# deepika090/HL-HGAT

Hardware: AMD Instinct MI355X
Metric: graphs/sec HL-HGAT fwd+bwd, ZINC-12k simplex graphs, 1/2/4/8 MI355X (higher is better)
Workload: dtype fp32; 1 GPU; BASELINE configs[1]: ZINC-12k-scale, HL_HGCNN_zinc_dense_int3_pyr channels=[2,2,2] filters=[64,64,64] K=3 mlp=[256,256] keig=15; step = copy of the device-resident batch into the step's static buffers + fwd + L1 + bwd (+ grad all-reduce) + Adam; the batch tables (Laplacian / incidence CSRs, degrees, segment offsets) are built by the data loader at collate time, outside the step (see loader); graphs_per_gpu=1000, global_batch=1000, parallelism=dp1

## Files before the change

hl-hgat_amd/csrc/collate.hip:

```cpp
#include <cstdint>
#include <cstring>
#include <vector>

#include "common.h"

namespace {

struct Sizes {
  int64_t n_t = 0, n_s = 0, z_t = 0, z_s = 0;
};

int batch_sizes(const hlhgat_packed_graphs_t* d, const int64_t* idx, int64_t B, Sizes& s) {
  for (int64_t b = 0; b < B; ++b) {
    const int64_t g = idx[b];
    HLH_CHECK_ARG(g >= 0 && g < d->n_graphs, "collate: graph id %lld out of range [0, %lld)",
                  (long long)g, (long long)d->n_graphs);
    s.n_t += d->node_ptr[g + 1] - d->node_ptr[g];
    s.n_s += d->edge_ptr[g + 1] - d->edge_ptr[g];
    s.z_t += d->lt_ptr[g + 1] - d->lt_ptr[g];
    s.z_s += d->ls_ptr[g + 1] - d->ls_ptr[g];
  }
  return HLHGAT_OK;
}

void pad_loops(int64_t n, int64_t R, int64_t z, int64_t Z, int64_t* row, int64_t* col,
               float* w) {
  const int64_t extra = Z - z, bins = R - n;
  if (extra <= 0 || bins <= 0) return;
  const int64_t base = extra / bins, more = extra % bins;
  int64_t p = z;
  for (int64_t r = n; r < R; ++r) {
    const int64_t k = base + (r - n < more ? 1 : 0);
    for (int64_t i = 0; i < k; ++i, ++p) {
      row[p] = r;
      col[p] = r;
      w[p] = 0.f;
    }
  }
}

void coo_csr(const int64_t* row, const int64_t* col, int64_t nnz, int64_t n, int32_t* rowptr,
             int32_t* ccol) {
  std::memset(rowptr, 0, sizeof(int32_t) * (size_t)(n + 1));
  for (int64_t e = 0; e < nnz; ++e) rowptr[row[e] + 1]++;
  for (int64_t r = 0; r < n; ++r) rowptr[r + 1] += rowptr[r];
  for (int64_t e = 0; e < nnz; ++e) ccol[e] = (int32_t)col[e];
}

}

extern "C" int hlhgat_collate_sizes(const hlhgat_packed_graphs_t* d, const int64_t* idx,
                                    int64_t n_idx, int64_t* sizes) {
  HLH_CHECK_ARG(d && sizes && n_idx >= 0 && (n_idx == 0 || idx), "collate_sizes: bad arguments");
  Sizes s;
  const int rc = batch_sizes(d, idx, n_idx, s);
  if (rc) return rc;
  sizes[0] = s.n_t;
  sizes[1] = s.n_s;
  sizes[2] = s.z_t;
  sizes[3] = s.z_s;
  return HLHGAT_OK;
}

extern "C" int hlhgat_collate(const hlhgat_packed_graphs_t* d, const int64_t* idx, int64_t B,
                              hlhgat_collated_t* o) {
  HLH_CHECK_ARG(d && o && B > 0 && idx, "collate: bad arguments");
  HLH_CHECK_ARG(d->node_ptr && d->edge_ptr && d->lt_ptr && d->ls_ptr && d->x_t && d->x_s &&
                    d->lt_row && d->lt_col && d->lt_w && d->ls_row && d->ls_col && d->ls_w &&
                    d->b1_src && d->b1_dst && d->f_t > 0 && d->f_s > 0 &&
                    (d->y_dim == 0 || d->y),
                "collate: incomplete packed dataset");
  Sizes s;
  int rc = batch_sizes(d, idx, B, s);
  if (rc) return rc;
  const int64_t Rt = o->rows_t, Rs = o->rows_s, Zt = o->nnz_t, Zs = o->nnz_s;
  const bool padded = !(Rt == s.n_t && Rs == s.n_s && Zt == s.z_t && Zs == s.z_s);
  if (padded)
    HLH_CHECK_ARG(Rt > s.n_t && Rs > s.n_s && Zt >= s.z_t && Zs >= s.z_s,
                  "collate: capacities (%lld, %lld, %lld, %lld) do not hold the batch "
                  "(%lld, %lld, %lld, %lld)",
                  (long long)Rt, (long long)Rs, (long long)Zt, (long long)Zs,
                  (long long)s.n_t, (long long)s.n_s, (long long)s.z_t, (long long)s.z_s);
  HLH_CHECK_ARG(Rt < INT32_MAX && 2 * Rs < INT32_MAX && Zt < INT32_MAX && Zs < INT32_MAX,
                "collate: batch too large for int32 tables");
  HLH_CHECK_ARG(o->x_t && o->x_s && o->edge_index_t && o->edge_weight_t && o->edge_index_s &&
                    o->edge_weight_s && o->edge_index && o->num_node1 && o->num_edge1 &&
                    (d->y_dim == 0 || o->y),
                "collate: NULL output");
  const int64_t Ft = d->f_t, Fs = d->f_s;
  int64_t* eit_r = o->edge_index_t;
  int64_t* eit_c = o->edge_index_t + Zt;
  int64_t* eis_r = o->edge_index_s;
  int64_t* eis_c = o->edge_index_s + Zs;
  int64_t* b1_r = o->edge_index;
  int64_t* b1_c = o->edge_index + Rs;
  int64_t nt = 0, ns = 0, zt = 0, zs = 0;
  for (int64_t b = 0; b < B; ++b) {
    const int64_t g = idx[b];
    const int64_t n0 = d->node_ptr[g], n1 = d->node_ptr[g + 1];
    const int64_t e0 = d->edge_ptr[g], e1 = d->edge_ptr[g + 1];
    const int64_t t0 = d->lt_ptr[g], t1 = d->lt_ptr[g + 1];
// ... 33 lines not shown
    }
    if (d->y_dim)
      std::memcpy(o->y + b * d->y_dim, d->y + g * d->y_dim, sizeof(float) * (size_t)d->y_dim);
    o->num_node1[b] = n1 - n0;
    o->num_edge1[b] = e1 - e0;
    nt += n1 - n0;
    ns += e1 - e0;
    zt += t1 - t0;
    zs += s1 - s0;
  }
  std::memset(o->x_t + nt * Ft, 0, sizeof(float) * (size_t)((Rt - nt) * Ft));
  std::memset(o->x_s + ns * Fs, 0, sizeof(float) * (size_t)((Rs - ns) * Fs));
  pad_loops(nt, Rt, zt, Zt, eit_r, eit_c, o->edge_weight_t);
  pad_loops(ns, Rs, zs, Zs, eis_r, eis_c, o->edge_weight_s);
  for (int64_t i = 0; i < Rs - ns; ++i) {
    b1_r[ns + i] = nt + i % (Rt - nt);
    b1_c[ns + i] = nt + i % (Rt - nt);
  }
  if (o->csr_rowptr_t && o->csr_col_t) coo_csr(eit_r, eit_c, Zt, Rt, o->csr_rowptr_t, o->csr_col_t);
  if (o->csr_rowptr_s && o->csr_col_s) coo_csr(eis_r, eis_c, Zs, Rs, o->csr_rowptr_s, o->csr_col_s);
  if (o->inc_rowptr && o->inc_eids) {
    int32_t* rp = o->inc_rowptr;
    std::memset(rp, 0, sizeof(int32_t) * (size_t)(Rt + 1));
    for (int64_t e = 0; e < Rs; ++e) {
      HLH_CHECK_ARG(b1_r[e] >= 0 && b1_r[e] < Rt && b1_c[e] >= 0 && b1_c[e] < Rt,
                    "collate: B1 edge %lld out of range", (long long)e);
      rp[b1_r[e] + 1]++;
      rp[b1_c[e] + 1]++;
    }
    for (int64_t r = 0; r < Rt; ++r) rp[r + 1] += rp[r];
    std::vector<int32_t> fill(rp, rp + Rt);
    for (int64_t e = 0; e < Rs; ++e) {
      o->inc_eids[fill[b1_r[e]]++] = (int32_t)e;
      o->inc_eids[fill[b1_c[e]]++] = (int32_t)e;
    }
    if (o->deg_t && o->inv_deg_t) {
      for (int64_t r = 0; r < Rt; ++r) {
        const float dv = (padded && r >= nt) ? 1.f : (float)(rp[r + 1] - rp[r]);
        o->deg_t[r] = dv;
        o->inv_deg_t[r] = 1.f / dv;
      }
    }
  }
  if (o->seg_ptr_t && o->seg_ptr_s) {
    o->seg_ptr_t[0] = 0;
    o->seg_ptr_s[0] = 0;
    for (int64_t b = 0; b < B; ++b) {
      o->seg_ptr_t[b + 1] = o->seg_ptr_t[b] + (int32_t)o->num_node1[b];
      o->seg_ptr_s[b + 1] = o->seg_ptr_s[b] + (int32_t)o->num_edge1[b];
    }
  }
  if (o->valid_mask_t)
    for (int64_t r = 0; r < Rt; ++r) o->valid_mask_t[r] = r < nt ? 1 : 0;
  o->n_t = nt;
  o->n_s = ns;
  return HLHGAT_OK;
}
```

hl-hgat_amd/csrc/poly.hip:

```cpp
#include "common.h"

#include <cstdlib>

using namespace hlhgat;

namespace {

struct PolyArgs {
  const int32_t* order;
  const int32_t* rowptr;
  const int32_t* col;
  const float* val;
  const float* rs;
  const float* X;
  const float* B;
  const float* Z;
  const float* P;
  const float* Q;
  float* Y;
  int64_t ldx, ldb, ldz, ldp, ldq, ldy;
  int64_t n_rows;
  int d;
  float alpha, beta, gamma, div, p, q;
  const int32_t* hdr;
// ... 117 lines not shown
            c[u] = __shfl(cm, j + u, LPR);
            w[u] = __shfl(wm, j + u, LPR);
          }
          if (fok) {
            vt x[8];
#pragma unroll
            for (int u = 0; u < 8; ++u) x[u] = vload<V>(X + (int64_t)c[u] * a.ldx + f);
#pragma unroll
            for (int i = 0; i < V; ++i) {
              float s = vget(acc, i);
#pragma unroll
              for (int u = 0; u < 8; ++u) s = s + w[u] * vget(x[u], i);
              vget(acc, i) = s;
            }
          }
        }
      }
      for (; j + 3 < cnt; j += 4) {
        const int c0 = __shfl(cm, j, LPR), c1 = __shfl(cm, j + 1, LPR),
                  c2 = __shfl(cm, j + 2, LPR), c3 = __shfl(cm, j + 3, LPR);
        const float w0 = __shfl(wm, j, LPR), w1 = __shfl(wm, j + 1, LPR),
                    w2 = __shfl(wm, j + 2, LPR), w3 = __shfl(wm, j + 3, LPR);
        if (fok) {
          vt x0 = vload<V>(X + (int64_t)c0 * a.ldx + f);
          vt x1 = vload<V>(X + (int64_t)c1 * a.ldx + f);
          vt x2 = vload<V>(X + (int64_t)c2 * a.ldx + f);
          vt x3 = vload<V>(X + (int64_t)c3 * a.ldx + f);
#pragma unroll
          for (int i = 0; i < V; ++i) {
            float s = vget(acc, i);
            s = s + w0 * vget(x0, i);
            s = s + w1 * vget(x1, i);
            s = s + w2 * vget(x2, i);
            s = s + w3 * vget(x3, i);
            vget(acc, i) = s;
          }
        }
      }
      if (j < cnt) gather_batch<V, 3, LPR>(X, a.ldx, f, fok, cm, wm, j, cnt - j, acc);
    }
    if (!fok) continue;
    poly_epilogue<V>(a, row, f, acc, rsv);
  }
}

template <int V, int LPR>
__global__ __launch_bounds__(256) void k_poly_step(PolyArgs a) {
  poly_step_body<V, LPR, 4>(a, blk_hw());
}

template <int V, int LPR>
__global__ __launch_bounds__(256) void k_poly_step_deep(PolyArgs a) {
  poly_step_body<V, LPR, 8>(a, blk_hw());
}

template <int V, int LPR>
__global__ __launch_bounds__(256) void k_hodge_edge_step(PolyArgs a) {
  using vt = typename VecT<V>::type;
  constexpr int kEpg = 4;
  const int64_t grp = ((int64_t)xcd_slot(blockIdx.x, gridDim.x) * 256 + threadIdx.x) / LPR;
  const int sub = threadIdx.x % LPR;
  const int64_t s0 = grp * kEpg;
  if (s0 >= a.n_rows) return;
  int64_t e[kEpg];
  int2 ij[kEpg];
  float al[kEpg];
#pragma unroll
  for (int u = 0; u < kEpg; ++u) {
    const int64_t sl = s0 + u < a.n_rows ? s0 + u : s0;
    e[u] = a.order ? (int64_t)a.order[sl] : sl;
  }
#pragma unroll
  for (int u = 0; u < kEpg; ++u) {
    ij[u] = a.ends[e[u]];
    al[u] = a.ealpha[e[u]];
  }
  const float* __restrict__ Z = a.X;
  for (int f = sub * V; f < a.d; f += LPR * V) {
    vt zi[kEpg], zj[kEpg];
#pragma unroll
    for (int u = 0; u < kEpg; ++u) {
      zi[u] = vload<V>(Z + (int64_t)ij[u].x * a.ldx + f);
      zj[u] = vload<V>(Z + (int64_t)ij[u].y * a.ldx + f);
    }
#pragma unroll
    for (int u = 0; u < kEpg; ++u) {
      if (s0 + u >= a.n_rows) break;
      vt acc;
#pragma unroll
      for (int c = 0; c < V; ++c) {
        float s = 0.f;
        s = s + (-al[u]) * vget(zi[u], c);
        s = s + al[u] * vget(zj[u], c);
        vget(acc, c) = s;
      }
      poly_epilogue<V>(a, e[u], f, acc, 1.f);
    }
  }
}

constexpr int kHaloIds = 8;

template <int V, int LPR, int NT>
__global__ __launch_bounds__(NT) void k_poly_halo(PolyArgs a) {
  using vt = typename VecT<V>::type;
  constexpr int FS = V * LPR;
// ... 454 lines not shown
}

int launch_factored(PolyArgs a, const hlhgat_hodge_factor_t& f, float* work, hipStream_t s) {
  HLH_CHECK_ARG(f.node_rowptr && f.ends && f.alpha && work && a.n_rows == f.n_edges &&
                    (f.n_edges == 0 || (f.node_edge && f.node_sign)),
                "hodge factor: incomplete descriptor or row count %lld != n_edges %lld",
                (long long)a.n_rows, (long long)f.n_edges);
  HLH_CHECK_ARG(!a.rs, "hodge factor: row scale not supported");
  if (a.n_rows == 0) return HLHGAT_OK;
  if (a.beta != 0.f && !a.B) {
    a.B = a.X;
    a.ldb = a.ldx;
  }
  {
    PolyArgs b = make_args(f.node_rowptr, f.node_edge, f.node_sign, f.n_nodes, a.X, a.ldx, a.d,
                           work, a.d, f.node_order);
    const double b1 = 16.0 * (double)f.n_edges + 4.0 * (double)(f.n_nodes + 1) +
                      4.0 * (double)(f.n_edges + f.n_nodes) * a.d;
    int rc = launch_poly(b, 2 * f.n_edges, s, HLHGAT_PROF_HODGE_NODE, b1);
    if (rc) return rc;
  }
  a.X = work;
  a.ldx = a.d;
  a.order = f.edge_order;
  a.ends = reinterpret_cast<const int2*>(f.ends);
  a.ealpha = f.alpha;
  a.lcol = nullptr;
  a.n_tiles = 0;
  const int v = pick_vec(a.d, {a.ldx, a.ldy, a.Z ? a.ldz : 4, a.P ? a.ldp : 4, a.Q ? a.ldq : 4,
                               a.B ? a.ldb : 4},
                         {a.X, a.Y, a.Z, a.P, a.Q, a.B});
  const int l = pick_lpr(a.d, v);
  a.nt_store = (double)a.n_rows * a.d * 4.0 >= kNtStoreBytes;
  int dense = 1 + (a.beta != 0.f) + (a.Z != nullptr) + (a.P != nullptr) + (a.Q != nullptr);
  ProfScope prof(HLHGAT_PROF_HODGE_EDGE, s,
                 12.0 * (double)a.n_rows + 4.0 * (double)(f.n_nodes + dense * a.n_rows) * a.d,
                 4.0 * (double)a.n_rows * a.d);
  HLH_DISPATCH_VL(v, l, k_hodge_edge_step, ceil_div(a.n_rows, (int64_t)4), s, a, &prof);
  HLH_CHECK_LAUNCH();
  return HLHGAT_OK;
}

struct StepRunner {
  int64_t nnz;
  const hlhgat_hodge_factor_t* fac;
  float* work;
  hipStream_t s;
  int prof_class = HLHGAT_PROF_POLY;
  int operator()(PolyArgs& a) const {
    return fac ? launch_factored(a, *fac, work, s) : launch_poly(a, nnz, s, prof_class);
  }
};

}

using namespace hlhgat;

extern "C" int hlhgat_spmm(const int32_t* rowptr, const int32_t* col,
                           const float* val, int64_t n_rows, int64_t nnz,
                           const int32_t* row_order, const hlhgat_halo_t* halo,
                           const float* X, int64_t ldx,
                           int64_t d, float* Y, int64_t ldy, void* stream) {
  PolyArgs a = make_args(rowptr, col, val, n_rows, X, ldx, d, Y, ldy, row_order, halo);
  return launch_poly(a, nnz, as_stream(stream));
}

extern "C" int hlhgat_poly_step(const int32_t* rowptr, const int32_t* col,
                                const float* val, const float* rs,
                                int64_t n_rows, int64_t nnz,
                                const int32_t* row_order, const hlhgat_halo_t* halo,
                                const float* X,
                                int64_t ldx, int64_t d, const float* Z,
                                int64_t ldz, const float* P, int64_t ldp,
                                const float* Q, int64_t ldq, float alpha,
                                float beta, float gamma, float div, float p,
                                float q, float* Y, int64_t ldy, void* stream) {
  PolyArgs a = make_args(rowptr, col, val, n_rows, X, ldx, d, Y, ldy, row_order, halo);
  a.rs = rs;
  a.Z = Z;
  a.ldz = ldz;
  a.P = P;
  a.ldp = ldp;
  a.Q = Q;
  a.ldq = ldq;
  a.alpha = alpha;
  a.beta = beta;
  a.gamma = gamma;
  a.div = div;
  a.p = p;
  a.q = q;
  return launch_poly(a, nnz, as_stream(stream));
}

extern "C" int hlhgat_incidence_step(const int32_t* rowptr, const int32_t* col,
                                     const float* val, const float* rs, int64_t n_rows,
                                     int64_t nnz, int64_t n_src, const float* X, int64_t ldx,
                                     int64_t d, const float* Z, int64_t ldz, float alpha,
                                     float gamma, float* Y, int64_t ldy, void* stream) {
  HLH_CHECK_ARG(n_src >= 0, "incidence_step: n_src < 0");
  PolyArgs a = make_args(rowptr, col, val, n_rows, X, ldx, d, Y, ldy);
  a.rs = rs;
  a.Z = Z;
  a.ldz = ldz;
  a.alpha = alpha;
  a.gamma = gamma;
  a.div = 1.f;
  const double bytes = (double)nnz * (val ? 8.0 : 4.0) + 4.0 * (double)(n_rows + 1) +
                       4.0 * (double)n_src * d + 4.0 * (double)n_rows * d * (Z ? 2.0 : 1.0) +
                       (rs ? 4.0 * (double)n_rows : 0.0);
  return launch_poly(a, nnz, as_stream(stream), HLHGAT_PROF_INCIDENCE, bytes);
}

namespace {
int basis_fwd_core(int kind, const int32_t* rowptr, const int32_t* col, const float* val,
                   int64_t n, int64_t nnz, const int32_t* row_order, const hlhgat_halo_t* halo,
                   const float* X, int64_t ldx, int64_t F, int K, float* T,
                   const hlhgat_hodge_factor_t* fac, float* work, void* stream) {
  HLH_CHECK_ARG(kind == HLHGAT_POLY_LAGUERRE || kind == HLHGAT_POLY_CHEB ||
                    kind == HLHGAT_POLY_LAGUERRE_DEMO,
                "poly_basis_fwd: bad kind %d", kind);
  HLH_CHECK_ARG(K >= 1, "poly_basis_fwd: K must be > 0 (assert K > 0)");
  if (K == 1 || n == 0) return HLHGAT_OK;
  HLH_CHECK_ARG(T, "poly_basis_fwd: T is NULL");
  hipStream_t s = as_stream(stream);
  const StepRunner run{nnz, fac, work, s};
  const int64_t blk = n * F;
  auto Tk = [&](int k) -> float* { return T + (int64_t)(k - 1) * blk; };
  {
    PolyArgs a = make_args(rowptr, col, val, n, X, ldx, F, Tk(1), F, row_order, halo);
    if (kind != HLHGAT_POLY_CHEB) {
      a.alpha = -1.f;
      a.beta = 1.f;
    }
    int rc = run(a);
    if (rc) return rc;
  }
  for (int k = 1; k + 1 < K; ++k) {
    const float* prev = (k == 1) ? X : Tk(k - 1);
    const int64_t ldprev = (k == 1) ? ldx : F;
    PolyArgs a = make_args(rowptr, col, val, n, Tk(k), F, F, Tk(k + 1), F, row_order, halo);
    a.Z = prev;
    a.ldz = ldprev;
    if (kind == HLHGAT_POLY_LAGUERRE_DEMO) {
      a.X = X;
      a.ldx = ldx;
      a.B = Tk(k);
      a.ldb = F;
      a.alpha = -1.f;
      a.beta = (float)(2 * k + 1);
      a.gamma = -(float)k;
      a.div = (float)(k + 1);
    } else if (kind == HLHGAT_POLY_LAGUERRE) {
      a.alpha = -1.f;
      a.beta = (float)(2 * k + 1);
      a.gamma = -(float)k;
      a.div = (float)(k + 1);
    } else {
      a.alpha = 2.f;
      a.gamma = -1.f;
    }
    int rc = run(a);
    if (rc) return rc;
  }
  return HLHGAT_OK;
}

int basis_bwd_core(int kind, const int32_t* rowptr_t, const int32_t* col_t,
                   const float* val_t, int64_t n, int64_t nnz, const int32_t* row_order,
                   const hlhgat_halo_t* halo, int64_t F, int K, float* G,
                   const hlhgat_hodge_factor_t* fac, float* work, void* stream) {
  HLH_CHECK_ARG(kind == HLHGAT_POLY_LAGUERRE || kind == HLHGAT_POLY_CHEB ||
                    kind == HLHGAT_POLY_LAGUERRE_DEMO,
                "poly_basis_bwd: bad kind %d", kind);
  HLH_CHECK_ARG(K >= 1, "poly_basis_bwd: K must be > 0");
  if (K == 1 || n == 0) return HLHGAT_OK;
  HLH_CHECK_ARG(G, "poly_basis_bwd: G is NULL");
  hipStream_t s = as_stream(stream);
  const StepRunner run{nnz, fac, work, s, HLHGAT_PROF_POLY_ADJ};
  const int64_t blk = n * F;
  auto Gk = [&](int k) -> float* { return G + (int64_t)k * blk; };
  if (kind == HLHGAT_POLY_LAGUERRE_DEMO) {
    HLH_CHECK_ARG(K <= DEMO_MAXK, "poly_basis_bwd: DEMO recurrence needs K <= %d", DEMO_MAXK);
    DemoArgs d{G, n * F, K};
    launch(k_demo_adjoint_fold, dim3((unsigned)ceil_div(n * F, (int64_t)256)), dim3(256), 0, s,
           nullptr, d);
    HLH_CHECK_LAUNCH();
    PolyArgs a = make_args(rowptr_t, col_t, val_t, n, Gk(1), F, F, Gk(0), F, row_order, halo);
    a.P = Gk(0);
    a.ldp = F;
    a.p = 1.f;
    return run(a);
  }
  for (int k = K - 1; k >= 1; --k) {
    PolyArgs a = make_args(rowptr_t, col_t, val_t, n, Gk(k), F, F, Gk(k - 1), F, row_order, halo);
    a.P = Gk(k - 1);
    a.ldp = F;
    a.p = 1.f;
    if (k + 1 <= K - 1) {
      a.Q = Gk(k + 1);
      a.ldq = F;
    }
    if (kind == HLHGAT_POLY_LAGUERRE) {
      a.alpha = -1.f;
      a.beta = (float)(2 * k - 1);
      a.div = (float)k;
      a.q = -(float)k / (float)(k + 1);
    } else {
      a.alpha = (k == 1) ? 1.f : 2.f;
      a.q = -1.f;
    }
    int rc = run(a);
    if (rc) return rc;
  }
  return HLHGAT_OK;
}

}

extern "C" int hlhgat_poly_basis_fwd(int kind, const int32_t* rowptr, const int32_t* col,
                                     const float* val, int64_t n, int64_t nnz,
                                     const int32_t* row_order, const hlhgat_halo_t* halo,
                                     const float* X, int64_t ldx, int64_t F, int K, float* T,
                                     void* stream) {
  return basis_fwd_core(kind, rowptr, col, val, n, nnz, row_order, halo, X, ldx, F, K, T,
                        nullptr, nullptr, stream);
}

extern "C" int hlhgat_poly_basis_bwd(int kind, const int32_t* rowptr_t, const int32_t* col_t,
                                     const float* val_t, int64_t n, int64_t nnz,
                                     const int32_t* row_order, const hlhgat_halo_t* halo,
                                     int64_t F, int K, float* G, void* stream) {
  return basis_bwd_core(kind, rowptr_t, col_t, val_t, n, nnz, row_order, halo, F, K, G,
                        nullptr, nullptr, stream);
}

extern "C" int64_t hlhgat_hodge_factor_work_floats(int64_t n_nodes, int64_t F) {
  return n_nodes > 0 && F > 0 ? n_nodes * F : 1;
}

extern "C" int hlhgat_hodge_spmm(const hlhgat_hodge_factor_t* f, const float* X, int64_t ldx,
                                 int64_t d, float* Y, int64_t ldy, float* work, void* stream) {
  HLH_CHECK_ARG(f, "hodge_spmm: NULL factor");
  HLH_CHECK_ARG(d > 0 && ldx >= d && ldy >= d && X && Y, "hodge_spmm: bad operands");
  PolyArgs a = make_args(nullptr, nullptr, nullptr, f->n_edges, X, ldx, d, Y, ldy);
  return launch_factored(a, *f, work, as_stream(stream));
}

extern "C" int hlhgat_hodge_poly_step(const hlhgat_hodge_factor_t* f, const float* X,
                                      int64_t ldx, int64_t d, const float* Z, int64_t ldz,
                                      const float* P, int64_t ldp, const float* Q, int64_t ldq,
                                      float alpha, float beta, float gamma, float div, float p,
                                      float q, float* Y, int64_t ldy, float* work, void* stream) {
  HLH_CHECK_ARG(f, "hodge_poly_step: NULL factor");
  HLH_CHECK_ARG(d > 0 && ldx >= d && ldy >= d && X && Y && (!Z || ldz >= d) &&
                    (!P || ldp >= d) && (!Q || ldq >= d) && div != 0.f,
                "hodge_poly_step: bad operands");
  PolyArgs a = make_args(nullptr, nullptr, nullptr, f->n_edges, X, ldx, d, Y, ldy);
  a.Z = Z;
  a.ldz = ldz;
  a.P = P;
  a.ldp = ldp;
  a.Q = Q;
  a.ldq = ldq;
  a.alpha = alpha;
  a.beta = beta;
  a.gamma = gamma;
  a.div = div;
  a.p = p;
  a.q = q;
  return launch_factored(a, *f, work, as_stream(stream));
}

extern "C" int hlhgat_poly_basis_fwd_factored(int kind, const hlhgat_hodge_factor_t* f,
                                              const float* X, int64_t ldx, int64_t F, int K,
                                              float* T, float* work, void* stream) {
  HLH_CHECK_ARG(f, "poly_basis_fwd_factored: NULL factor");
  return basis_fwd_core(kind, nullptr, nullptr, nullptr, f->n_edges, 0, nullptr, nullptr, X, ldx,
                        F, K, T, f, work, stream);
}

extern "C" int hlhgat_poly_basis_bwd_factored(int kind, const hlhgat_hodge_factor_t* f,
                                              int64_t F, int K, float* G, float* work,
                                              void* stream) {
  HLH_CHECK_ARG(f, "poly_basis_bwd_factored: NULL factor");
  return basis_bwd_core(kind, nullptr, nullptr, nullptr, f->n_edges, 0, nullptr, nullptr, F, K,
                        G, f, work, stream);
// ... 101 lines not shown
```

hl-hgat_amd/csrc/runtime.hip:

```cpp
#include "common.h"

#include <cstring>
#include <mutex>
#include <vector>

namespace hlhgat {

static thread_local std::string g_last_error;

void set_error(const char* fmt, ...) {
  char buf[1024];
  va_list ap;
  va_start(ap, fmt);
  vsnprintf(buf, sizeof(buf), fmt, ap);
  va_end(ap);
  g_last_error = buf;
}

namespace {
constexpr int kPoolSize = 1 << 14;
struct ProfClass {
  bool enabled = false;
  std::vector<hipEvent_t> start, stop;
  std::vector<double> bytes, flops;
  int used = 0;
  int64_t dropped = 0;
};
std::mutex g_prof_mu;
ProfClass g_prof[HLHGAT_PROF_NCLASS];
}

ProfScope::ProfScope(int kernel_class, hipStream_t s, double b, double f)
    : cls(kernel_class), bytes(b), flops(f) {
  (void)s;
  if (kernel_class < 0 || kernel_class >= HLHGAT_PROF_NCLASS) return;
  std::lock_guard<std::mutex> lk(g_prof_mu);
  ProfClass& pc = g_prof[kernel_class];
  if (!pc.enabled) return;
  if (pc.used >= (int)pc.start.size()) {
    pc.dropped++;
    return;
  }
  slot = pc.used++;
  pc.bytes[slot] = b;
  pc.flops[slot] = f;
  start_ev = pc.start[slot];
  stop_ev = pc.stop[slot];
}

namespace {
std::mutex g_err_mu;
unsigned* g_err_word = nullptr;
}

unsigned* device_error_word() {
  std::lock_guard<std::mutex> lk(g_err_mu);
  if (!g_err_word) {
    void* p = nullptr;
    hipError_t e = hipHostMalloc(&p, 64, hipHostMallocPortable | hipHostMallocMapped |
                                             hipHostMallocCoherent);
    if (e != hipSuccess) {
      set_error("hipHostMalloc(device error word) failed: %s", hipGetErrorString(e));
      return nullptr;
    }
    *static_cast<volatile unsigned*>(p) = 0u;
    g_err_word = static_cast<unsigned*>(p);
  }
  return g_err_word;
}

}

using namespace hlhgat;

extern "C" int hlhgat_version(void) { return 107; }

extern "C" int hlhgat_device_errors(unsigned* out) {
  HLH_CHECK_ARG(out, "device_errors: NULL pointer");
  unsigned* w = device_error_word();
  HLH_CHECK_ARG(w, "device_errors: %s", hlhgat_last_error());
  *out = *static_cast<volatile unsigned*>(w);
  return HLHGAT_OK;
}

extern "C" int hlhgat_clear_device_errors(void) {
  unsigned* w = device_error_word();
  HLH_CHECK_ARG(w, "clear_device_errors: %s", hlhgat_last_error());
  *static_cast<volatile unsigned*>(w) = 0u;
  return HLHGAT_OK;
}

extern "C" const char* hlhgat_last_error(void) { return g_last_error.c_str(); }

extern "C" int hlhgat_stream_create(int device, unsigned flags, int priority,
                                    const uint32_t* cu_mask, int cu_mask_words, void** out) {
  HLH_CHECK_ARG(out && device >= 0 && cu_mask_words >= 0 && (cu_mask_words == 0 || cu_mask) &&
                    (cu_mask_words == 0 || priority == 0),
                "stream_create: bad arguments (a CU-masked stream has the default priority)");
  int prev = 0;
  HLH_CHECK_HIP(hipGetDevice(&prev));
  HLH_CHECK_HIP(hipSetDevice(device));
  hipStream_t s = nullptr;
  hipError_t e;
  if (cu_mask_words > 0) {
    int cus = 0;
    e = hipDeviceGetAttribute(&cus, hipDeviceAttributeMultiprocessorCount, device);
    int on = 0;
    for (int w = 0; w < cu_mask_words; ++w) on += __builtin_popcount(cu_mask[w]);
    if (e == hipSuccess && (on == 0 || cu_mask_words * 32 < cus)) {
      (void)hipSetDevice(prev);
      HLH_CHECK_ARG(false, "stream_create: the CU mask must cover all %d CUs (%d words given) "
                    "and enable at least one", cus, cu_mask_words);
    }
    if (e == hipSuccess) e = hipExtStreamCreateWithCUMask(&s, (uint32_t)cu_mask_words, cu_mask);
  } else if (priority != 0) {
    e = hipStreamCreateWithPriority(&s, flags, priority);
  } else {
    e = hipStreamCreateWithFlags(&s, flags);
  }
  (void)hipSetDevice(prev);
  HLH_CHECK_HIP(e);
  *out = s;
  return HLHGAT_OK;
}

extern "C" int hlhgat_stream_cu_mask(void* stream, uint32_t* cu_mask, int cu_mask_words) {
  HLH_CHECK_ARG(stream && cu_mask && cu_mask_words > 0, "stream_cu_mask: bad arguments");
  HLH_CHECK_HIP(hipExtStreamGetCUMask(as_stream(stream), (uint32_t)cu_mask_words, cu_mask));
// ... 421 lines not shown
```

hl-hgat_amd/csrc/torch_ext.cpp:

```cpp
#include <torch/extension.h>
#include <c10/hip/HIPStream.h>
#include <ATen/hip/impl/HIPGuardImplMasqueradingAsCUDA.h>
#include <ATen/hip/impl/HIPStreamMasqueradingAsCUDA.h>

#include <algorithm>
#include <cstring>
#include <mutex>
#include <optional>
#include <type_traits>
#include <unordered_map>
#include <unordered_set>
#include <vector>

#include "../../include/hlhgat.h"

namespace {

using torch::Tensor;
using torch::autograd::AutogradContext;
using torch::autograd::variable_list;
using OptT = std::optional<Tensor>;

inline void* stream_of(const Tensor& t) {
  return c10::hip::getCurrentHIPStream(t.get_device()).stream();
// ... 533 lines not shown
    return *streams;
  }
  static TStream side_of(int dev) {
    auto& streams = registry();
    auto it = streams.find(dev);
    if (it == streams.end()) {
      c10::hip::HIPGuardMasqueradingAsCUDA g((c10::DeviceIndex)dev);
      hipStream_t raw = nullptr;
      TORCH_CHECK(hipStreamCreateWithFlags(&raw, hipStreamNonBlocking) == hipSuccess,
                  "hlhgat: hipStreamCreateWithFlags");
      it = streams.emplace(dev, c10::hip::getStreamFromExternalMasqueradingAsCUDA(
                                    raw, (c10::DeviceIndex)dev)).first;
    }
    return it->second;
  }
  static hipEvent_t next_event() {
    static thread_local std::vector<hipEvent_t> pool;
    static thread_local size_t k = 0;
    if (pool.empty()) {
      pool.resize(64);
      for (auto& e : pool) TORCH_CHECK(hipEventCreateWithFlags(&e, hipEventDisableTiming) == 0);
    }
    return pool[k++ % pool.size()];
  }
  static void order(const TStream& from, const TStream& to) {
    hipEvent_t e = next_event();
    TORCH_CHECK(hipEventRecord(e, from.stream()) == hipSuccess, "hlhgat: hipEventRecord");
    TORCH_CHECK(hipStreamWaitEvent(to.stream(), e, 0) == hipSuccess, "hlhgat: hipStreamWaitEvent");
  }
  void side_waits_main() { order(main, side); }
  void main_waits_side() { order(side, main); }
  void escape(std::initializer_list<Tensor> ts) {
    for (const auto& t : ts)
      if (t.defined()) t.record_stream(main);
  }
};

struct ConvArgs {
  Tensor x, a_rowptr, a_col;
  OptT a_val;
  Tensor t_rowptr, t_col;
  OptT t_val;
  int64_t nnz = 0, kind = 0;
  std::vector<Tensor> W;
  OptT bias, bn_w, bn_b, bn_rm, bn_rv, bn_nbt;
  double momentum = 0.1, eps = 1e-5;
  int64_t bn_mode = 0;
  OptT out_buf, a_order, t_order;
  OptT valid, h_tile, h_ptr, h_cols, h_srp, h_lcol, h_sval;
  std::vector<int64_t> h_bounds;
  OptT h_hdr;
  std::vector<Tensor> fac;
  int64_t fac_nodes = 0;
};

struct ConvDims {
  int64_t N, Cin, F, M, dout, K, kind, nnz, bn_mode, fac_nodes;
};
struct ConvSaved {
  Tensor x2, T, t_order, valid, t_rowptr, t_col, t_val, pre, yout, mean, invstd, bn_w, bias,
      bn_b, h_tile, h_ptr, h_cols, h_srp, h_lcol, h_sval, h_hdr;
  std::vector<Tensor> W, fac;
  ConvDims d{};
  std::vector<int64_t> xshape, h_bounds;
  std::vector<Tensor*> slots() {
    return {&x2, &T, &t_order, &valid, &t_rowptr, &t_col, &t_val, &pre, &yout, &mean, &invstd,
            &bn_w, &bias, &bn_b, &h_tile, &h_ptr, &h_cols, &h_srp, &h_lcol, &h_sval, &h_hdr};
  }
  void save(AutogradContext* ctx) {
    ctx->saved_data["dims"] = pod_ints(d);
    ctx->saved_data["xshape"] = xshape;
    ctx->saved_data["h_bounds"] = h_bounds;
    std::vector<Tensor> tail = W;
    tail.insert(tail.end(), fac.begin(), fac.end());
    save_slots(ctx, *this, tail);
  }
  static ConvSaved load(AutogradContext* ctx) {
    ConvSaved s;
    s.d = ints_pod<ConvDims>(ctx->saved_data["dims"].toIntVector());
    s.xshape = ctx->saved_data["xshape"].toIntVector();
    s.h_bounds = ctx->saved_data["h_bounds"].toIntVector();
    s.fac = load_slots(ctx, s);
    s.W.assign(s.fac.begin(), s.fac.begin() + s.d.K);
    s.fac.erase(s.fac.begin(), s.fac.begin() + s.d.K);
    return s;
  }
};

struct ConvPos {
  int64_t x, W0, bias, bn_w, bn_b;
};
ConvPos walk_conv(EdgeMap& em, const ConvArgs& c) {
  ConvPos p;
  p.x = em.tensor();
  em.tensor(2);
  em.opt(c.a_val);
  em.tensor(2);
  em.opt(c.t_val);
  em.other(2);
  p.W0 = em.list(c.W);
  p.bias = em.opt(c.bias);
  p.bn_w = em.opt(c.bn_w);
  p.bn_b = em.opt(c.bn_b);
  em.opt(c.bn_rm);
  em.opt(c.bn_rv);
  em.opt(c.bn_nbt);
  em.other(3);
  em.opt(c.out_buf);
  em.opt(c.a_order);
  em.opt(c.t_order);
  em.opt(c.valid);
  em.opt(c.h_tile);
  em.opt(c.h_ptr);
  em.opt(c.h_cols);
  em.opt(c.h_srp);
  em.opt(c.h_lcol);
  em.opt(c.h_sval);
  em.other();
  em.opt(c.h_hdr);
  em.list(c.fac);
  em.other();
  return p;
}

Tensor conv_forward(const ConvArgs& c, ConvSaved& sv) {
  const Tensor& x = c.x;
  req(x, "x");
  const int64_t N = x.size(0);
  const int64_t Cin = x.size(-1);
  const int64_t K = (int64_t)c.W.size();
  Tensor x2 = x.dim() == 2 ? rows2d(x) : x.contiguous().view({N, -1});
  const int64_t F = x2.size(1);
  const int64_t M = N * (F / Cin);
  const int64_t dout = c.W[0].size(0);
  void* s = stream_of(x);
  Tensor T = at::empty({std::max<int64_t>(K - 1, 0), N, F}, x.options());
  const bool use_halo = has(c.h_lcol) && has(c.h_tile) && has(c.h_ptr) && has(c.h_cols) &&
                        has(c.h_srp) && has(c.h_hdr);
  const hlhgat_halo_t halo =
      use_halo ? make_halo(*c.h_tile, *c.h_ptr, *c.h_cols, *c.h_srp, *c.h_lcol,
                           has(c.h_sval) ? *c.h_sval : Tensor(), c.h_bounds, *c.h_hdr)
               : hlhgat_halo_t{};
  const bool factored = !c.fac.empty();
  if (factored && K > 1 && N > 0) {
    const hlhgat_hodge_factor_t hf = make_factor(c.fac, c.fac_nodes, N);
    Tensor work = at::empty({hlhgat_hodge_factor_work_floats(c.fac_nodes, F)}, x.options());
    chk(hlhgat_poly_basis_fwd_factored((int)c.kind, &hf, x2.data_ptr<float>(), ld_of(x2), F,
                                       (int)K, T.data_ptr<float>(), work.data_ptr<float>(), s),
        "poly_basis_fwd_factored");
  } else if (K > 1 && N > 0) {
    chk(hlhgat_poly_basis_fwd((int)c.kind, c.a_rowptr.data_ptr<int>(),
                              c.nnz ? c.a_col.data_ptr<int>() : nullptr,
                              c.nnz ? fptr(c.a_val) : nullptr, N, c.nnz, iptr(c.a_order),
                              use_halo ? &halo : nullptr, x2.data_ptr<float>(), ld_of(x2), F, (int)K, T.data_ptr<float>(), s),
        "poly_basis_fwd");
  }
  std::vector<const float*> Ap(K), Wp(K);
  std::vector<int64_t> lda(K), ldw(K), kb(K, Cin);
  Ap[0] = x2.data_ptr<float>();
  lda[0] = x.dim() == 2 ? ld_of(x2) : Cin;
  for (int64_t k = 1; k < K; ++k) {
    Ap[k] = T.data_ptr<float>() + (k - 1) * N * F;
    lda[k] = Cin;
  }
  for (int64_t k = 0; k < K; ++k) {
    req(c.W[k], "lins[k].weight");
    TORCH_CHECK(c.W[k].stride(1) == 1, "hlhgat: weights need unit inner stride");
    Wp[k] = c.W[k].data_ptr<float>();
    ldw[k] = c.W[k].stride(0);
  }
  const bool sink = has(c.out_buf);
  if (sink)
    TORCH_CHECK(c.out_buf->size(0) == M && c.out_buf->size(1) == dout &&
                    c.out_buf->stride(1) == 1 && c.out_buf->device() == x.device(),
                "hlhgat: conv output buffer must be a row-major [", M, ", ", dout, "] view");
  Tensor pre = (sink && c.bn_mode == 0) ? *c.out_buf : at::empty({M, dout}, x.options());
  Tensor out = pre;
  const BnState st{c.bn_w, c.bn_b, c.bn_rm, c.bn_rv, c.bn_nbt, c.momentum, c.eps, c.valid};
  if (M > 0 && c.bn_mode > 0) {
    out = proj_bn_forward(Ap, lda, Wp, ldw, kb, M, dout, fptr(c.bias), pre, st, c.bn_mode == 2,
                          sv.mean, sv.invstd, sink ? &*c.out_buf : nullptr);
  } else {
    if (M > 0) {
      proj_fwd(Ap, lda, Wp, ldw, kb, M, dout, fptr(c.bias), pre, s);
    } else if (has(c.bias)) {
      pre.copy_(c.bias->expand_as(pre));
    }
    if (c.bn_mode > 0)
      out = bn_forward(pre, st, c.bn_mode == 2, sv.mean, sv.invstd,
                       sink ? &*c.out_buf : nullptr);
  }
  sv.d = {N, Cin, F, M, dout, K, c.kind, c.nnz, c.bn_mode, c.fac_nodes};
  sv.h_bounds = c.h_bounds;
  sv.xshape = x.sizes().vec();
  sv.x2 = x2;
  sv.T = T;
  sv.t_order = opt_or_undef(c.t_order);
  sv.valid = opt_or_undef(c.valid);
  sv.t_rowptr = c.t_rowptr;
  sv.t_col = c.t_col;
  sv.t_val = opt_or_undef(c.t_val);
  if (c.bn_mode > 0) sv.pre = pre;
  if (c.bn_mode == 2) sv.yout = out;
  sv.bn_w = opt_or_undef(c.bn_w);
  sv.bias = opt_or_undef(c.bias);
  sv.bn_b = opt_or_undef(c.bn_b);
  if (use_halo && c.t_rowptr.data_ptr() == c.a_rowptr.data_ptr()) {
    sv.h_tile = *c.h_tile;
    sv.h_ptr = *c.h_ptr;
    sv.h_cols = *c.h_cols;
    sv.h_srp = *c.h_srp;
    sv.h_lcol = *c.h_lcol;
    sv.h_sval = opt_or_undef(c.h_sval);
    sv.h_hdr = *c.h_hdr;
  }
  sv.W = c.W;
  sv.fac = c.fac;
  std::vector<int64_t> oshape = x.sizes().vec();
  oshape.back() = dout;
  return out.view(oshape);
}

variable_list conv_backward(const ConvSaved& sv, const Tensor& grad, const Edges<ConvPos>& ed) {
  const ConvDims& d = sv.d;
  const ConvPos& pos = ed.pos;
  const int64_t N = d.N, Cin = d.Cin, F = d.F, M = d.M, K = d.K;
  const Tensor& x2 = sv.x2;
  const bool use_halo = sv.h_lcol.defined();
  const hlhgat_halo_t halo =
      use_halo ? make_halo(sv.h_tile, sv.h_ptr, sv.h_cols, sv.h_srp, sv.h_lcol, sv.h_sval,
                           sv.h_bounds, sv.h_hdr)
               : hlhgat_halo_t{};
  void* s = stream_of(x2);
  Tensor G = rows2d(grad.reshape({M, d.dout}));
  variable_list out = ed.grads();
  const bool need_x = ed.need(pos.x);
  bool need_w = false;
  for (int64_t k = 0; k < K; ++k) need_w = need_w || ed.need(pos.W0 + k);
  const bool need_b = ed.need(pos.bias);
  if (d.bn_mode > 0) {
    const OptT bn_y = d.bn_mode == 2 ? OptT(sv.yout) : OptT();
    G = bn_backward(sv.pre, bn_y, G, undef_to_opt(sv.bn_w), sv.mean, sv.invstd,
                    ed.need(pos.bn_w), ed.need(pos.bn_b), out[pos.bn_w], out[pos.bn_b], nullptr,
                    &sv.bn_b, sv.valid);
  }
  GradW gw;
  if (need_w || need_b) {
    gw.A.resize(K);
    gw.lda = gw.kb = gw.lddw = std::vector<int64_t>(K, Cin);
    gw.A[0] = x2.data_ptr<float>();
    if (sv.xshape.size() == 2) gw.lda[0] = ld_of(x2);
    for (int64_t k = 1; k < K; ++k) gw.A[k] = sv.T.data_ptr<float>() + (k - 1) * N * F;
    for (int64_t k = 0; k < K; ++k) {
      const bool nk = ed.need(pos.W0 + k);
      gw.out.push_back(nk ? grad_like(sv.W[k]) : at::empty({d.dout, Cin}, x2.options()));
      gw.dW.push_back(gw.out[k].data_ptr<float>());
      if (nk) out[pos.W0 + k] = gw.out[k];
    }
    if (need_b) {
      out[pos.bias] = grad_like(sv.bias);
      gw.db = out[pos.bias].data_ptr<float>();
      gw.out.push_back(out[pos.bias]);
    }
  }
  GradD gd;
  Tensor Gs;
  if (need_x) {
    Gs = at::empty({K, N, F}, x2.options());
    gd.kb = gd.ldda = std::vector<int64_t>(K, Cin);
    for (int64_t k = 0; k < K; ++k) {
      gd.W.push_back(sv.W[k].data_ptr<float>());
      gd.ldw.push_back(sv.W[k].stride(0));
      gd.dA.push_back(Gs.data_ptr<float>() + k * N * F);
    }
  }
  linear_grads(G, (need_w || need_b) ? &gw : nullptr, need_x ? &gd : nullptr, s);
  if (need_x) {
    if (M > 0 && K > 1 && !sv.fac.empty()) {
      const hlhgat_hodge_factor_t hf = make_factor(sv.fac, d.fac_nodes, N);
      Tensor work = at::empty({hlhgat_hodge_factor_work_floats(d.fac_nodes, F)}, x2.options());
      chk(hlhgat_poly_basis_bwd_factored((int)d.kind, &hf, F, (int)K, Gs.data_ptr<float>(),
                                         work.data_ptr<float>(), s),
          "poly_basis_bwd_factored");
    } else if (M > 0 && K > 1) {
      const Tensor &tv = sv.t_val, &to = sv.t_order;
      chk(hlhgat_poly_basis_bwd((int)d.kind, sv.t_rowptr.data_ptr<int>(),
                                d.nnz ? sv.t_col.data_ptr<int>() : nullptr,
                                (d.nnz && tv.defined()) ? tv.data_ptr<float>() : nullptr, N, d.nnz,
                                to.defined() ? to.data_ptr<int>() : nullptr,
                                use_halo ? &halo : nullptr, F, (int)K, Gs.data_ptr<float>(), s),
          "poly_basis_bwd");
    } else if (M == 0) {
      Gs.zero_();
    }
    out[pos.x] = Gs[0].view(sv.xshape);
  }
  return out;
}

class ConvBNFn : public torch::autograd::Function<ConvBNFn> {
 public:
  static Tensor forward(AutogradContext* ctx, Tensor x, Tensor a_rowptr, Tensor a_col,
                        OptT a_val, Tensor t_rowptr, Tensor t_col, OptT t_val, int64_t nnz,
                        int64_t kind, at::TensorList W, OptT bias, OptT bn_w, OptT bn_b,
                        OptT bn_rm, OptT bn_rv, OptT bn_nbt, double momentum, double eps,
                        int64_t bn_mode, OptT out_buf, OptT a_order, OptT t_order, OptT valid,
                        OptT h_tile, OptT h_ptr, OptT h_cols, OptT h_srp, OptT h_lcol,
                        OptT h_sval, std::vector<int64_t> h_bounds, OptT h_hdr,
                        at::TensorList fac, int64_t fac_nodes) {
    ConvArgs c{x, a_rowptr, a_col, a_val, t_rowptr, t_col, t_val, nnz, kind, W.vec(), bias,
               bn_w, bn_b, bn_rm, bn_rv, bn_nbt, momentum, eps, bn_mode, out_buf, a_order,
               t_order, valid, h_tile, h_ptr, h_cols, h_srp, h_lcol, h_sval, h_bounds, h_hdr,
               fac.vec(), fac_nodes};
    ConvSaved sv;
    Tensor y = conv_forward(c, sv);
    EdgeMap em;
    save_edges(ctx, em, walk_conv(em, c));
    sv.save(ctx);
    return y;
  }

  static variable_list backward(AutogradContext* ctx, variable_list grads) {
    return conv_backward(ConvSaved::load(ctx), grads[0], Edges<ConvPos>(ctx));
  }
};

class BNActFn : public torch::autograd::Function<BNActFn> {
 public:
  struct Pos {
    int64_t x, w, b;
  };
  struct Saved {
    Tensor x, y, w, mean, invstd, b, valid;
    std::vector<Tensor*> slots() { return {&x, &y, &w, &mean, &invstd, &b, &valid}; }
  };
  static Tensor forward(AutogradContext* ctx, Tensor x, OptT w, OptT b, OptT rm, OptT rv,
                        OptT nbt, double momentum, double eps, bool relu, OptT valid) {
    req(x, "x");
    Saved sv;
    sv.x = rows2d(x);
    Tensor y = bn_forward(sv.x, BnState{w, b, rm, rv, nbt, momentum, eps, valid}, relu, sv.mean,
                          sv.invstd);
    EdgeMap em;
    const Pos pos{em.tensor(), em.opt(w), em.opt(b)};
    em.opt(rm);
    em.opt(rv);
    em.opt(nbt);
    em.other(3);
    em.opt(valid);
    save_edges(ctx, em, pos);
    if (relu) sv.y = y;
    sv.w = opt_or_undef(w);
    sv.b = opt_or_undef(b);
    sv.valid = opt_or_undef(valid);
    save_slots(ctx, sv);
    return y;
  }
  static variable_list backward(AutogradContext* ctx, variable_list grads) {
    Saved sv;
    load_slots(ctx, sv);
    const Edges<Pos> ed(ctx);
    const Pos& pos = ed.pos;
    variable_list out = ed.grads();
    out[pos.x] = bn_backward(sv.x, undef_to_opt(sv.y), grads[0], undef_to_opt(sv.w), sv.mean,
                             sv.invstd, ed.need(pos.w), ed.need(pos.b), out[pos.w], out[pos.b],
                             nullptr, &sv.b, sv.valid);
// ... 739 lines not shown
                    state.is_contiguous(), "hlhgat: dropout state must be two int64 on the device");
    if (has(out))
      TORCH_CHECK(out->dim() == 2 && out->size(0) == n && out->size(1) == d &&
                      out->stride(1) == 1 && out->stride(0) >= d && out->device() == x.device() &&
                      out->scalar_type() == at::kFloat,
                  "hlhgat: dropout out must be a [", n, ", ", d, "] row-strided fp32 block");
    Tensor y = has(out) ? *out : at::empty({n, d}, xs.options());
    Tensor snap = at::empty({2}, state.options());
    chk(hlhgat_dropout_fwd(xs.data_ptr<float>(), ld_of(xs), n, d, (uint32_t)T, (float)s,
                           state.data_ptr<int64_t>(), (uint32_t)site, snap.data_ptr<int64_t>(),
                           y.data_ptr<float>(), ld_of(y), stream_of(xs)),
        "dropout_fwd");
    ctx->saved_data["T"] = T;
    ctx->saved_data["s"] = s;
    ctx->saved_data["site"] = site;
    EdgeMap em;
    const Pos pos{em.tensor()};
    em.other(2);
    em.tensor();
    em.other();
    em.opt(out);
    save_edges(ctx, em, pos);
    ctx->save_for_backward({snap});
    return y;
  }
  static variable_list backward(AutogradContext* ctx, variable_list grads) {
    const Tensor snap = ctx->get_saved_variables().front();
    const Edges<Pos> ed(ctx);
    Tensor g = rows2d(grads[0]);
    const int64_t n = g.size(0), d = g.size(1);
    Tensor gx = at::empty({n, d}, g.options());
    chk(hlhgat_dropout_bwd(g.data_ptr<float>(), ld_of(g), n, d,
                           (uint32_t)ctx->saved_data["T"].toInt(),
                           (float)ctx->saved_data["s"].toDouble(), snap.data_ptr<int64_t>(),
                           (uint32_t)ctx->saved_data["site"].toInt(), gx.data_ptr<float>(),
                           ld_of(gx), stream_of(g)),
        "dropout_bwd");
    variable_list grads_in = ed.grads();
    grads_in[ed.pos.x] = gx;
    return grads_in;
  }
};

Tensor hip_dropout(Tensor x, int64_t T, double s, Tensor state, int64_t site, OptT out) {
  return DropoutFn::apply(x, T, s, state, site, out);
}

Tensor conv_bn(Tensor x, Tensor a_rowptr, Tensor a_col, OptT a_val, Tensor t_rowptr, Tensor t_col,
               OptT t_val, int64_t nnz, int64_t kind, std::vector<Tensor> W, OptT bias, OptT bn_w,
               OptT bn_b, OptT bn_rm, OptT bn_rv, OptT bn_nbt, double momentum, double eps,
               int64_t bn_mode, OptT out_buf, OptT a_order, OptT t_order, OptT valid,
               OptT h_tile, OptT h_ptr, OptT h_cols, OptT h_srp, OptT h_lcol, OptT h_sval,
               std::vector<int64_t> h_bounds, OptT h_hdr, std::vector<Tensor> fac,
               int64_t fac_nodes) {
  return ConvBNFn::apply(x, a_rowptr, a_col, a_val, t_rowptr, t_col, t_val, nnz, kind,
                         at::TensorList(W), bias, bn_w, bn_b, bn_rm, bn_rv, bn_nbt, momentum, eps,
                         bn_mode, out_buf, a_order, t_order, valid, h_tile, h_ptr, h_cols, h_srp, h_lcol, h_sval, h_bounds,
                         h_hdr, at::TensorList(fac), fac_nodes);
}

Tensor bn_act(Tensor x, OptT w, OptT b, OptT rm, OptT rv, OptT nbt, double momentum, double eps,
              bool relu, OptT valid) {
  return BNActFn::apply(x, w, b, rm, rv, nbt, momentum, eps, relu, valid);
}

Tensor linear(std::vector<Tensor> As, Tensor W, OptT b) {
  return LinearFn::apply(W, b, at::TensorList(As));
}

Tensor mlp2(std::vector<Tensor> blocks, Tensor W0, OptT b0, OptT g1, OptT be1, OptT rm1, OptT rv1,
            OptT nbt1, Tensor W3, OptT b3, OptT g4, OptT be4, OptT rm4, OptT rv4, OptT nbt4,
            double mom1, double eps1, double mom4, double eps4) {
  return MLP2Fn::apply(at::TensorList(blocks), W0, b0, g1, be1, rm1, rv1, nbt1, W3, b3, g4, be4,
                       rm4, rv4, nbt4, mom1, eps1, mom4, eps4);
}

Tensor node_from_edges(Tensor x_s, Tensor rowptr, Tensor eids, Tensor ei, Tensor rD,
                       int64_t n_nodes) {
  return NodeFromEdgesFn::apply(x_s, rowptr, eids, ei, rD, n_nodes);
}

Tensor edge_from_nodes(Tensor x_t, Tensor rowptr, Tensor eids, Tensor ei) {
  return EdgeFromNodesFn::apply(x_t, rowptr, eids, ei);
}

std::vector<Tensor> nei_value(Tensor x_t, Tensor x_s, Tensor rowptr, Tensor eids, Tensor ei,
                              Tensor rD, std::vector<Tensor> pn, std::vector<Tensor> pe,
                              double mom1n, double eps1n, double mom4n, double eps4n,
                              double mom1e, double eps1e, double mom4e, double eps4e,
                              OptT valid_t, OptT valid_s, OptT gsink_t, OptT gsink_s,
                              OptT gflag_t, OptT gflag_s, OptT packed) {
  auto r = NEIntValueFn::apply(x_t, x_s, rowptr, eids, ei, rD, at::TensorList(pn),
                               at::TensorList(pe), mom1n, eps1n, mom4n, eps4n, mom1e, eps1e,
                               mom4e, eps4e, valid_t, valid_s, gsink_t, gsink_s, gflag_t,
                               gflag_s, packed);
  return {r[0], r[1]};
}


inline void req_i32(const Tensor& t, const char* name) {
  TORCH_CHECK(t.is_cuda() && t.scalar_type() == at::kInt && t.dim() == 1 && t.is_contiguous(),
              "hlhgat: ", name, " must be a contiguous int32 1-D ROCm tensor");
}
inline void req_csr(const Tensor& rowptr, const Tensor& col, const OptT& val) {
  req_i32(rowptr, "rowptr");
  req_i32(col, "col");
  TORCH_CHECK(rowptr.numel() >= 1, "hlhgat: rowptr needs n_rows + 1 >= 1 entries");
  TORCH_CHECK(col.numel() < ((int64_t)1 << 31), "hlhgat: nnz must be < 2^31");
  if (has(val))
    TORCH_CHECK(val->is_cuda() && val->scalar_type() == at::kFloat && val->is_contiguous() &&
                    val->numel() == col.numel(),
// ... 477 lines not shown
```

hl-hgat_amd/hlhgat/_lib.py:

```python
from __future__ import annotations

import ctypes as C
import os

import torch

_HERE = os.path.dirname(os.path.abspath(__file__))
LIB_PATH = os.environ.get("HLHGAT_LIB", os.path.join(_HERE, "libhlhgat.so"))

c_i32, c_i64, c_f32, c_f64, c_vp, c_sz = (C.c_int32, C.c_int64, C.c_float,
                                           C.c_double, C.c_void_p, C.c_size_t)
P_i64 = C.POINTER(c_i64)
P_i32 = C.POINTER(c_i32)
P_f64 = C.POINTER(c_f64)
P_vp = C.POINTER(c_vp)

MAX_COPY_BLOCKS = 64

SIGNATURES = {
    "hlhgat_version": (c_i32, []),
    "hlhgat_last_error": (C.c_char_p, []),
    "hlhgat_csr_workspace_bytes": (c_sz, [c_i64]),
    "hlhgat_csr_from_coo": (c_i32, [c_vp, c_vp, c_vp, c_i64, c_i64, c_i64, c_vp, c_vp,
                                    c_vp, c_vp, c_vp, c_sz, c_vp]),
    "hlhgat_csr_from_sorted_coo": (c_i32, [c_vp, c_vp, c_vp, c_i64, c_i64, c_vp, c_vp,
                                           c_vp, c_vp]),
    "hlhgat_coo_check_sorted": (c_i32, [c_vp, c_vp, c_i64, c_i64, c_i64, c_vp, c_vp]),
    "hlhgat_incidence_csr": (c_i32, [c_vp, c_i64, c_i64, c_vp, c_vp, c_vp, c_sz, c_vp]),
    "hlhgat_halo_tiles": (c_i32, [c_vp, c_vp, c_i64, c_i64, c_vp, c_i32, c_i32, c_i32, c_vp,
                                  c_vp, c_vp, c_vp, c_vp, c_vp, c_vp, P_i64, P_i64]),
    "hlhgat_graclus": (c_i32, [c_vp, c_vp, c_i64, c_i64, c_vp, c_vp]),
    "hlhgat_mlgc_map": (c_i32, [c_vp, c_i64, c_vp, c_i64, c_vp, c_vp, c_vp, P_i64, P_i64]),
    "hlhgat_mlgc_batch": (c_i32, [c_i64, c_vp, c_vp, c_vp, c_vp, c_i32, c_vp, c_vp, c_vp, c_vp,
                                  c_vp]),
    "hlhgat_gather_f32": (c_i32, [c_vp, c_vp, c_i64, c_vp, c_vp]),
    "hlhgat_collate_sizes": (c_i32, [c_vp, c_vp, c_i64, c_vp]),
    "hlhgat_collate": (c_i32, [c_vp, c_vp, c_i64, c_vp]),
    "hlhgat_spmm": (c_i32, [c_vp, c_vp, c_vp, c_i64, c_i64, c_vp, c_vp, c_vp, c_i64, c_i64,
                            c_vp, c_i64, c_vp]),
    "hlhgat_poly_step": (c_i32, [c_vp, c_vp, c_vp, c_vp, c_i64, c_i64, c_vp, c_vp, c_vp,
                                 c_i64, c_i64, c_vp, c_i64, c_vp, c_i64, c_vp, c_i64, c_f32,
                                 c_f32, c_f32, c_f32, c_f32, c_f32, c_vp, c_i64, c_vp]),
    "hlhgat_incidence_step": (c_i32, [c_vp, c_vp, c_vp, c_vp, c_i64, c_i64, c_i64, c_vp, c_i64,
                                      c_i64, c_vp, c_i64, c_f32, c_f32, c_vp, c_i64, c_vp]),
    "hlhgat_poly_basis_fwd": (c_i32, [c_i32, c_vp, c_vp, c_vp, c_i64, c_i64, c_vp, c_vp,
                                      c_vp, c_i64, c_i64, c_i32, c_vp, c_vp]),
    "hlhgat_poly_basis_bwd": (c_i32, [c_i32, c_vp, c_vp, c_vp, c_i64, c_i64, c_vp, c_vp,
                                      c_i64, c_i32, c_vp, c_vp]),
    "hlhgat_hodge_factor_work_floats": (c_i64, [c_i64, c_i64]),
    "hlhgat_hodge_spmm": (c_i32, [c_vp, c_vp, c_i64, c_i64, c_vp, c_i64, c_vp, c_vp]),
    "hlhgat_hodge_poly_step": (c_i32, [c_vp, c_vp, c_i64, c_i64, c_vp, c_i64, c_vp, c_i64, c_vp,
                                       c_i64, c_f32, c_f32, c_f32, c_f32, c_f32, c_f32, c_vp,
                                       c_i64, c_vp, c_vp]),
    "hlhgat_poly_basis_fwd_factored": (c_i32, [c_i32, c_vp, c_vp, c_i64, c_i64, c_i32, c_vp,
                                               c_vp, c_vp]),
    "hlhgat_poly_basis_bwd_factored": (c_i32, [c_i32, c_vp, c_i64, c_i32, c_vp, c_vp, c_vp]),
    "hlhgat_hodge_lmax_workspace_bytes": (c_i64, [c_i64, c_i32]),
    "hlhgat_hodge_lmax": (c_i32, [c_vp, c_vp, c_vp, c_i64, c_i64, c_vp, c_i64, c_i32, c_vp, c_vp,
                                  c_i64, c_vp]),
    "hlhgat_bn_bwd_reduce": (c_i32, [c_vp, c_i64, c_vp, c_i64, c_vp, c_i64, c_i64, c_vp, c_i64,
                                     c_vp, c_vp, c_vp, c_vp, c_vp, c_vp, c_vp, c_i64, c_vp]),
    "hlhgat_eig_pe_workspace_bytes": (c_i64, [c_i64, c_i64, c_i32]),
    "hlhgat_eig_pe": (c_i32, [c_vp, c_vp, c_vp, c_i64, c_i64, c_vp, c_i64, c_i64, c_i32, c_vp,
                              c_i64, c_vp, c_vp, c_i64, c_vp]),
    "hlhgat_hodge_row_sizes": (c_i32, [c_vp, c_vp, c_i64, c_i64, c_vp, c_vp, c_vp]),
    "hlhgat_hodge_build": (c_i32, [c_vp, c_vp, c_vp, c_i64, c_i64, c_vp, c_vp, c_vp, c_vp, c_i64,
                                   c_vp, c_vp, c_vp, c_i64, c_vp]),
    "hlhgat_proj_fwd": (c_i32, [c_i32, P_vp, P_i64, P_vp, P_i64, P_i64, c_i64, c_i64, c_vp,
                                c_vp, c_i64, c_i32, c_vp]),
    "hlhgat_proj_bwd_data": (c_i32, [c_i32, c_vp, c_i64, P_vp, P_i64, P_i64, c_i64, c_i64,
                                     P_vp, P_i64, c_i32, c_vp]),
    "hlhgat_proj_bwd_weight_workspace_floats": (c_i64, [c_i32, P_i64, c_i64, c_i64, c_i32]),
    "hlhgat_proj_bwd_weight": (c_i32, [c_i32, c_vp, c_i64, P_vp, P_i64, P_i64, c_i64, c_i64,
                                       P_vp, P_i64, c_vp, c_i32, c_vp, c_i64, c_vp]),
    "hlhgat_proj_bwd": (c_i32, [c_i64, c_i64, c_vp, c_i64, c_i32, P_vp, P_i64, P_i64, P_vp,
                                P_i64, c_vp, c_i32, P_vp, P_i64, P_i64, P_vp, P_i64, c_i32,
                                c_vp, c_i64, c_vp]),
    "hlhgat_proj_bwd_defer": (c_i32, [c_i64, c_i64, c_vp, c_i64, c_i32, P_vp, P_i64, P_i64,
                                      P_vp, P_i64, c_vp, c_i32, P_vp, P_i64, P_i64, P_vp, P_i64,
                                      c_i32, c_vp, c_i64, c_vp, c_vp, c_vp, c_vp]),
    "hlhgat_reduce_run": (c_i32, [c_vp, c_vp]),
    "hlhgat_proj_bn_fwd": (c_i32, [c_i32, P_vp, P_i64, P_vp, P_i64, P_i64, c_i64, c_i64, c_vp,
                                   c_vp, c_i64, c_vp, c_vp, c_vp, c_vp, c_vp, c_vp, c_f32,
                                   c_f32, c_i32, c_vp, c_i64, c_vp, c_vp, c_vp, c_i64, c_vp]),
    "hlhgat_set_proj_bn_fused": (c_i32, [c_i32]),
    "hlhgat_set_proj_bn_split": (c_i32, [c_i32]),
    "hlhgat_set_proj_bwd_rows": (c_i32, [c_i32]),
    "hlhgat_set_gemm_big": (c_i32, [c_i32, c_i64]),
    "hlhgat_proj_bn_fused_capacity": (c_i32, [P_i64]),
    "hlhgat_set_bn_one_launch": (c_i32, [c_i32]),
    "hlhgat_get_bn_one_launch": (c_i32, []),
    "hlhgat_set_bn_bwd_one_launch": (c_i32, [c_i32]),
    "hlhgat_get_bn_bwd_one_launch": (c_i32, []),
    "hlhgat_set_bn_wait_us": (c_i32, [C.c_uint32]),
    "hlhgat_set_proj_bn_stamps": (c_i32, [c_vp, c_i64]),
    "hlhgat_bn_giveup_log": (c_i32, [c_vp, c_i32, c_vp]),
    "hlhgat_bn_giveup_reset": (c_i32, []),
    "hlhgat_test_occupy": (c_i32, [c_i32, c_i32, c_i32, C.c_uint32, c_vp]),
    "hlhgat_device_errors": (c_i32, [c_vp]),
    "hlhgat_stream_create": (c_i32, [c_i32, C.c_uint32, c_i32, c_vp, c_i32, c_vp]),
    "hlhgat_stream_cu_mask": (c_i32, [c_vp, c_vp, c_i32]),
# ... 102 lines not shown
    "hlhgat_leaky_maxpool_time_bwd": (c_i32, [c_vp, c_vp, c_vp, c_i64, c_i64, c_i64, c_i32,
                                              c_f32, c_vp, c_vp]),
    "hlhgat_time_readout_fwd": (c_i32, [c_vp, c_i64, c_i64, c_i64, c_f32, c_vp, c_vp, c_vp]),
    "hlhgat_time_readout_bwd": (c_i32, [c_vp, c_vp, c_vp, c_i64, c_i64, c_i64, c_f32, c_vp,
                                        c_vp]),
    "hlhgat_fc_workspace_bytes": (c_sz, [c_i64, c_i64, c_i64]),
    "hlhgat_fc_prepare": (c_i32, [c_vp, c_i64, c_vp, c_i64, c_i64, c_i64, c_i64, c_vp, c_vp,
                                  c_sz, c_vp]),
    "hlhgat_fc_dense": (c_i32, [c_vp, c_i64, c_i64, c_i64, c_vp, c_vp]),
    "hlhgat_fc_edges": (c_i32, [c_vp, c_i64, c_i64, c_i64, c_vp, c_i64, c_vp, c_i64, c_vp,
                                c_i64, c_vp]),
}

POLY_LAGUERRE, POLY_CHEB, POLY_LAGUERRE_DEMO = 0, 1, 2
SIGMA_SIGMOID, SIGMA_RELU = 0, 1
DEVERR_BN_STATE = 1
DEVERR_HODGE_SIZE = 2
DEVERR_LABEL = 4
DEVERR_METRIC_LABEL = 8
DEVERR_METER_FULL = 16
DEVERR_EIGPE_SIZE = 32
LOSS_MEAN, LOSS_SUM, LOSS_FOCAL = 0, 1, 2
CE_MAX_CLASSES = 64
LOSS_ONE_LAUNCH_MAX = 16384
BN_LOG_MAX = 64
PROF_POLY, PROF_PROJ, PROF_HODGE_NODE, PROF_HODGE_EDGE = 0, 1, 2, 3
PROF_PROJ_BWD, PROF_BN_FWD, PROF_BN_BWD, PROF_PROJ_BN = 4, 5, 6, 7
PROF_POLY_ADJ, PROF_INCIDENCE, PROF_GATHER2 = 8, 9, 10
MAX_BLOCKS = 16


class BnGiveup(C.Structure):
    _fields_ = [(f, C.c_uint32) for f in ("kernel", "tile", "block", "total", "arrivals", "gen0",
                                          "gen_seen", "wait_us", "outcome")]


class HaloDesc(C.Structure):
    _fields_ = [("hdr", c_vp), ("tile_ptr", c_vp), ("halo_ptr", c_vp), ("halo", c_vp), ("srp", c_vp),
                ("lcol", c_vp), ("sval", c_vp), ("n_tiles", c_i64), ("max_halo", c_i32),
                ("max_rows", c_i32), ("max_nnz", c_i32)]


class HodgeFactorDesc(C.Structure):
    _fields_ = [("node_rowptr", c_vp), ("node_edge", c_vp), ("node_sign", c_vp),
                ("node_order", c_vp), ("n_nodes", c_i64), ("ends", c_vp), ("alpha", c_vp),
                ("edge_order", c_vp), ("n_edges", c_i64)]


class PackedGraphsDesc(C.Structure):
    _fields_ = [("n_graphs", c_i64), ("node_ptr", c_vp), ("edge_ptr", c_vp), ("lt_ptr", c_vp),
                ("ls_ptr", c_vp), ("x_t", c_vp), ("f_t", c_i64), ("x_s", c_vp), ("f_s", c_i64),
                ("lt_row", c_vp), ("lt_col", c_vp), ("lt_w", c_vp), ("ls_row", c_vp),
                ("ls_col", c_vp), ("ls_w", c_vp), ("b1_src", c_vp), ("b1_dst", c_vp),
                ("y", c_vp), ("y_dim", c_i64)]


class CollatedDesc(C.Structure):
    _fields_ = [("rows_t", c_i64), ("rows_s", c_i64), ("nnz_t", c_i64), ("nnz_s", c_i64),
                ("x_t", c_vp), ("x_s", c_vp), ("edge_index_t", c_vp), ("edge_weight_t", c_vp),
                ("edge_index_s", c_vp), ("edge_weight_s", c_vp), ("edge_index", c_vp),
                ("y", c_vp), ("num_node1", c_vp), ("num_edge1", c_vp), ("csr_rowptr_t", c_vp),
                ("csr_col_t", c_vp), ("csr_rowptr_s", c_vp), ("csr_col_s", c_vp),
                ("inc_rowptr", c_vp), ("inc_eids", c_vp), ("deg_t", c_vp), ("inv_deg_t", c_vp),
                ("seg_ptr_t", c_vp), ("seg_ptr_s", c_vp), ("valid_mask_t", c_vp),
                ("n_t", c_i64), ("n_s", c_i64)]


class HlhgatError(RuntimeError):
    pass


def load(path: str = LIB_PATH) -> C.CDLL:
    if not os.path.exists(path):
        raise ImportError(
            f"hlhgat: HIP library not found at {path}. Build it with "
            f"`python -c 'import __graft_entry__ as g; g.build()'` or "
            f"`make -C hl-hgat_amd/csrc` (hipcc --offload-arch=gfx950).")
    lib = C.CDLL(path, mode=C.RTLD_GLOBAL)
    for name, (res, args) in SIGNATURES.items():
        fn = getattr(lib, name)
        fn.restype = res
        fn.argtypes = args
    return lib


LIB = load()


def check(rc: int, what: str) -> None:
    if rc != 0:
        msg = LIB.hlhgat_last_error().decode(errors="replace")
        raise HlhgatError(f"{what} failed (code {rc}): {msg}")
```

hl-hgat_amd/hlhgat/hodge_dataset.py:

```python
from __future__ import annotations

from typing import Dict, List, Optional, Sequence, Tuple

import os

import numpy as np
import torch

__all__ = ["PairData", "Batch", "collate", "adj2par1", "BoundaryOperator", "degree",
           "hodge_laplacians", "dense_to_sparse", "is_sorted_symmetric", "locality_order",
           "static_caps", "pad_batch", "level_caps", "pad_levels", "PackedGraphs", "halo_tiles", "graclus", "mlgc", "mlgc_weighted", "mlgc_map", "to_undirected_mean",
           "hodge_factor_ok", "hodge_coo_from_boundary", "fc2mask"]

_INC_KEYS = ("edge_index_s", "edge_index_t", "edge_index", "row_order_s", "row_order_t")
_HODGE_KEYS = ("edge_index_s", "edge_index_t")


class PairData:

    def __init__(self, edge_index_s=None, x_s=None, edge_index_t=None, x_t=None,
                 edge_weight_s=None, edge_weight_t=None, edge_index=None, y=None, **kw):
        self.edge_index_s = edge_index_s
        self.x_s = x_s
        self.edge_index_t = edge_index_t
# ... 40 lines not shown
        for k in self.keys():
            v = getattr(self, k)
            if torch.is_tensor(v):
                setattr(self, k, v.to(device, non_blocking=non_blocking))
        self._mark()
        return self

    def _check_counts(self) -> None:
        for kc, kx in (("num_node1", "x_t"), ("num_edge1", "x_s")):
            c, x = getattr(self, kc, None), getattr(self, kx, None)
            if torch.is_tensor(c) and torch.is_tensor(x) and not c.is_cuda:
                tot = int(c.sum())
                if tot > x.shape[0]:
                    raise ValueError(f"Batch.{kc} sums to {tot} but {kx} has "
                                     f"{x.shape[0]} rows")

    def _mark(self) -> None:
        from . import ops
        from .ops import mark_hodge, set_halo, set_row_order, set_valid
        for k, ok in (getattr(self, "hodge_sorted", None) or {}).items():
            t = getattr(self, k, None)
            if ok and torch.is_tensor(t) and t.is_cuda:
                mark_hodge(t)
        for k, ko, kv in (("edge_index_s", "row_order_s", "n_valid_s"),
                          ("edge_index_t", "row_order_t", "n_valid_t")):
            t, o = getattr(self, k, None), getattr(self, ko, None)
            nv = getattr(self, kv, None)
            if torch.is_tensor(t) and t.is_cuda and torch.is_tensor(o):
                set_row_order(t, o)
            if torch.is_tensor(t) and t.is_cuda and torch.is_tensor(nv):
                set_valid(t, nv)
            side = k[-1]
            hk = {h: getattr(self, h + "_" + side, None) for h in _HALO_KEYS + ("halo_bounds",)}
            if (torch.is_tensor(t) and t.is_cuda and all(torch.is_tensor(v) for v in hk.values())
                    and self.hodge_sorted.get(k, False)):
                set_halo(t, hk)
        ei = getattr(self, "edge_index", None)
        eis = getattr(self, "edge_index_s", None)
        if (getattr(self, "l1_factor", False) and torch.is_tensor(ei) and ei.is_cuda
                and torch.is_tensor(eis) and eis.is_cuda):
            tabs = tuple(getattr(self, k, None) for k in ("fac_alpha", "fac_sign", "fac_ends"))
            tabs = tabs if all(torch.is_tensor(t) and t.is_cuda for t in tabs) else None
            ops.set_hodge_factor(eis, ei, self.x_t.size(0), getattr(self, "row_order_t", None),
                                 tables=tabs)
            if tabs is not None:
                ei._hlhgat_inc_signs = tabs[1]
        for side in ("t", "s"):
            k = "edge_index_" + side
            t = getattr(self, k, None)
            rp, col = getattr(self, "csr_rowptr_" + side, None), getattr(self, "csr_col_" + side, None)
            if (torch.is_tensor(t) and t.is_cuda and torch.is_tensor(rp) and torch.is_tensor(col)
                    and self.hodge_sorted.get(k, False)):
                ops.set_csr(t, rp, col)
        ip, ie = getattr(self, "inc_rowptr", None), getattr(self, "inc_eids", None)
        if torch.is_tensor(ei) and ei.is_cuda and torch.is_tensor(ip) and torch.is_tensor(ie):
            ops.set_incidence(ei, ip, ie)
        dg, rdg = getattr(self, "deg_t", None), getattr(self, "inv_deg_t", None)
        if torch.is_tensor(dg) and dg.is_cuda and torch.is_tensor(rdg):
            dg._hlhgat_rcp = rdg
        if torch.is_tensor(ei) and ei.is_cuda:
            for kv in ("n_valid_t", "n_valid_s"):
                nv = getattr(self, kv, None)
                if torch.is_tensor(nv):
                    set_valid(ei, nv, "_hlhgat_valid_" + kv[-1])

    @property
    def batch_t(self) -> torch.Tensor:
        return torch.repeat_interleave(torch.arange(self.num_graphs, device=self.x_t.device),
                                       self.num_node1.to(self.x_t.device))

    @property
    def batch_s(self) -> torch.Tensor:
        return torch.repeat_interleave(torch.arange(self.num_graphs, device=self.x_s.device),
                                       self.num_edge1.to(self.x_s.device))


def locality_order(edge_index, n: int) -> torch.Tensor:
    import scipy.sparse as sp
    from scipy.sparse.csgraph import reverse_cuthill_mckee
    ei = np.asarray(edge_index)
    A = sp.csr_matrix((np.ones(ei.shape[1], dtype=np.int8), (ei[0], ei[1])), shape=(n, n))
    return torch.from_numpy(reverse_cuthill_mckee(A, symmetric_mode=True).astype(np.int64))


HALO_MAX = 160
HALO_ROWS = 24
HALO_NNZ = 768
_HALO_KEYS = ("halo_tile_ptr", "halo_ptr", "halo", "halo_srp", "halo_lcol", "halo_eperm",
              "halo_hdr")


def halo_tiles(edge_index, n: int, order=None, max_rows: int = HALO_ROWS,
               max_halo: int = HALO_MAX, max_nnz: int = HALO_NNZ
               ) -> Optional[Dict[str, torch.Tensor]]:
    import ctypes as C
    from ._lib import LIB
    ei = np.asarray(edge_index)
    nnz = ei.shape[1]
    rowptr = np.zeros(n + 1, dtype=np.int32)
    np.cumsum(np.bincount(ei[0], minlength=n), out=rowptr[1:])
    col = np.ascontiguousarray(ei[1], dtype=np.int32)
    ordr = None if order is None else np.ascontiguousarray(np.asarray(order), dtype=np.int32)
    tile_ptr = np.zeros(n + 1, dtype=np.int32)
    halo_ptr = np.zeros(n + 1, dtype=np.int32)
    srp = np.zeros(n + 1, dtype=np.int32)
    halo = np.zeros(max(nnz, 1), dtype=np.int32)
# ... 42 lines not shown
        roff += getattr(g, xk).size(0)
        hoff += int(ghp[-1])
        eoff += int(np.asarray(getattr(g, ek)).shape[1])
    for k, parts in zip(keys, (tp, hp, hc, srp, lc, ep, hd)):
        setattr(b, k, torch.from_numpy(np.ascontiguousarray(np.concatenate(parts))))
    setattr(b, bk, torch.from_numpy(bounds.copy()))


def is_sorted_symmetric(ei: np.ndarray, w: Optional[np.ndarray]) -> bool:
    if ei.shape[1] == 0:
        return True
    r, c = ei[0], ei[1]
    if np.any((r[1:] < r[:-1]) | ((r[1:] == r[:-1]) & (c[1:] < c[:-1]))):
        return False
    order = np.lexsort((r, c))
    if not (np.array_equal(c[order], r) and np.array_equal(r[order], c)):
        return False
    if w is not None and not np.array_equal(w[order], w):
        return False
    return True


def incidence_csr(edge_index, n_nodes: int) -> Tuple[torch.Tensor, torch.Tensor]:
    ei = np.asarray(edge_index, dtype=np.int64).reshape(2, -1)
    E = ei.shape[1]
    if E and (ei.min() < 0 or ei.max() >= n_nodes):
        raise ValueError(f"incidence_csr: node index out of range [0, {n_nodes})")
    e = np.arange(E, dtype=np.int64)
    keys = np.sort(np.concatenate([ei[0] * E + e, ei[1] * E + e]), kind="stable")
    rowptr = np.zeros(n_nodes + 1, dtype=np.int32)
    if E:
        np.cumsum(np.bincount(keys // E, minlength=n_nodes), out=rowptr[1:])
    return (torch.from_numpy(rowptr),
            torch.from_numpy((keys % E if E else keys).astype(np.int32)))


def laplacian_csr(edge_index, n: int) -> Tuple[torch.Tensor, torch.Tensor]:
    ei = np.asarray(edge_index, dtype=np.int64).reshape(2, -1)
    rowptr = np.zeros(n + 1, dtype=np.int32)
    if ei.shape[1]:
        np.cumsum(np.bincount(ei[0], minlength=n)[:n], out=rowptr[1:])
    return torch.from_numpy(rowptr), torch.from_numpy(ei[1].astype(np.int32))


def _attach_csr(b, sides=("t", "s")) -> None:
    for side in sides:
        k = "edge_index_" + side
        ei, x = getattr(b, k, None), getattr(b, "x_" + side, None)
        if torch.is_tensor(ei) and torch.is_tensor(x) and (getattr(b, "hodge_sorted", None)
                                                            or {}).get(k, False):
            rp, col = laplacian_csr(ei, x.size(0))
            setattr(b, "csr_rowptr_" + side, rp)
            setattr(b, "csr_col_" + side, col)


FACTOR_TABLES = os.environ.get("HLHGAT_FACTOR_TABLES", "1") != "0"


def factor_tables(b) -> None:
    ei_s = np.asarray(b.edge_index_s, dtype=np.int64)
    w = np.asarray(b.edge_weight_s, dtype=np.float32)
    E = int(b.x_s.shape[0])
    diag = ei_s[0] == ei_s[1]
    alpha = np.zeros(E, dtype=np.float32)
    np.add.at(alpha, ei_s[0][diag], w[diag] * np.float32(0.5))
    rp = np.asarray(b.inc_rowptr, dtype=np.int64)
    eids = np.asarray(b.inc_eids, dtype=np.int64)
    ei = np.asarray(b.edge_index, dtype=np.int64).reshape(2, -1)
    node = np.repeat(np.arange(rp.size - 1, dtype=np.int64), np.diff(rp))
    sign = np.where(ei[1][eids] == node, np.float32(1.0), np.float32(-1.0)).astype(np.float32)
    b.fac_alpha = torch.from_numpy(alpha)
    b.fac_sign = torch.from_numpy(np.ascontiguousarray(sign))
    b.fac_ends = torch.from_numpy(np.ascontiguousarray(ei.T.astype(np.int32)))


def node_degree(inc_rowptr: torch.Tensor, valid: Optional[int] = None
                ) -> Tuple[torch.Tensor, torch.Tensor]:
    rp = np.asarray(inc_rowptr, dtype=np.int64)
    d = (rp[1:] - rp[:-1]).astype(np.float32)
    if valid is not None:
        d[valid:] = 1.0
    with np.errstate(divide="ignore"):
        r = np.float32(1.0) / d
    return torch.from_numpy(d), torch.from_numpy(r.astype(np.float32))


def collate(graphs: Sequence[PairData], check_hodge: bool = True) -> Batch:
    b = Batch()
    B = len(graphs)
    b.num_graphs = B
    first = graphs[0]
    keys = first.keys()
    for k in keys:
        if k.rsplit("_", 1)[0] in _HALO_KEYS + ("halo_bounds",):
            continue
        vals = [getattr(g, k) for g in graphs]
        v0 = vals[0]
        if k in _INC_KEYS:
            incs = np.array([g.__inc__(k) for g in graphs], dtype=np.int64)
            off = np.concatenate([[0], np.cumsum(incs)[:-1]])
            cat = np.concatenate([np.asarray(v) + o for v, o in zip(vals, off)], axis=-1)
            setattr(b, k, torch.from_numpy(np.ascontiguousarray(cat)))
        elif torch.is_tensor(v0):
            if v0.dim() == 0:
                setattr(b, k, torch.stack(vals))
            else:
                setattr(b, k, torch.cat(vals, dim=0))
        elif isinstance(v0, (int, np.integer, float)):
            setattr(b, k, torch.tensor(vals))
        else:
            setattr(b, k, vals)
    b.num_nodes = int(sum(g.x_t.size(0) for g in graphs))
    hs = {}
    for k, wk in (("edge_index_s", "edge_weight_s"), ("edge_index_t", "edge_weight_t")):
        if getattr(b, k, None) is None:
            continue
        if check_hodge:
            ok = all(is_sorted_symmetric(np.asarray(getattr(g, k)),
                                         None if getattr(g, wk, None) is None
                                         else np.asarray(getattr(g, wk)))
                     for g in graphs)
        else:
            ok = all(getattr(g, "_hodge_sorted", False) for g in graphs)
        hs[k] = ok
    b.hodge_sorted = hs
    b.l1_factor = bool(hs.get("edge_index_s")) and _factor_wanted(graphs)
    for side in ("s", "t"):
        _collate_halo(b, graphs, side)
    _attach_csr(b)
    ei = getattr(b, "edge_index", None)
    if torch.is_tensor(ei) and torch.is_tensor(getattr(b, "x_t", None)):
        b.inc_rowptr, b.inc_eids = incidence_csr(ei, b.x_t.size(0))
        b.deg_t, b.inv_deg_t = node_degree(b.inc_rowptr)
        if b.l1_factor and FACTOR_TABLES:
            factor_tables(b)
    for key, ck in (("seg_ptr_t", "num_node1"), ("seg_ptr_s", "num_edge1")):
        c = getattr(b, ck, None)
        if torch.is_tensor(c) and c.dim() == 1 and not c.is_floating_point():
            ptr = torch.zeros(c.numel() + 1, dtype=torch.int32)
            ptr[1:] = torch.cumsum(c, 0).to(torch.int32)
            setattr(b, key, ptr)
    return b


FACTOR_MIN_ROW = 8.0


def hodge_factor_ok(edge_index, n_nodes: int, edge_index_s, edge_weight_s) -> bool:
    ei = np.asarray(edge_index)
    eis = np.asarray(edge_index_s)
    w = np.asarray(edge_weight_s, dtype=np.float32).reshape(-1)
    E = ei.shape[1] if ei.ndim == 2 else 0
    if E == 0 or eis.shape[1] != w.size or np.any(ei[0] >= ei[1]):
        return False
    r, c = eis[0], eis[1]
    if r.min() < 0 or max(r.max(), c.max()) >= E:
        return False
    diag = r == c
    if int(diag.sum()) != E or not np.array_equal(np.sort(r[diag]), np.arange(E)):
        return False
    alpha = np.zeros(E, dtype=np.float32)
    alpha[r[diag]] = w[diag] * np.float32(0.5)
    a, b, p, q = ei[0][r], ei[1][r], ei[0][c], ei[1][c]
    if np.any(~diag & (a == p) & (b == q)):
        return False
    v = np.where(diag, 2, np.where((a == p) | (b == q), 1, np.where((a == q) | (b == p), -1, 0)))
    if np.any(v == 0) or not np.array_equal(w, alpha[r] * v.astype(np.float32)):
        return False
    deg = np.bincount(ei.reshape(-1), minlength=int(n_nodes)).astype(np.int64)
    if eis.shape[1] != E + int((deg * (deg - 1)).sum()):
        return False
    key = r.astype(np.int64) * E + c
    return np.unique(key).size == key.size


def _factor_wanted(graphs) -> bool:
    E = sum(int(np.asarray(g.edge_index_s).shape[1]) for g in graphs)
    rows = sum(int(g.x_s.shape[0]) for g in graphs)
    if rows == 0 or E < FACTOR_MIN_ROW * rows:
        return False
    for g in graphs:
        ok = getattr(g, "_l1_factor_ok", None)
        if ok is None:
            if getattr(g, "edge_index", None) is None or getattr(g, "edge_weight_s", None) is None:
                return False
            ok = hodge_factor_ok(g.edge_index, g.x_t.shape[0], g.edge_index_s, g.edge_weight_s)
            g._l1_factor_ok = ok
        if not ok:
            return False
    return True


PAD_MIN_ROWS = 64


def _spread(n_items: int, n_bins: int) -> np.ndarray:
    base, extra = divmod(int(n_items), int(n_bins))
    return np.full(n_bins, base, dtype=np.int64) + (np.arange(n_bins) < extra)


def _roundup(v: int, q: int) -> int:
    return (int(v) + q - 1) // q * q


def static_caps(b: "Batch", quantum: int = 512) -> Dict[str, int]:
    rows_t = _roundup(b.x_t.size(0) + PAD_MIN_ROWS, quantum)
    rows_s = _roundup(b.x_s.size(0) + PAD_MIN_ROWS, quantum)
    caps = {"rows_t": rows_t, "rows_s": rows_s,
            "nnz_t": _roundup(b.edge_index_t.size(1) + 1, 4 * quantum),
            "nnz_s": _roundup(b.edge_index_s.size(1) + 1, 4 * quantum)}
    return caps


def pool_tables(datas: Sequence["Batch"], pos: bool = False) -> None:
    pairs = list(zip(datas[:-1], datas[1:])) if pos else [(datas[0], datas[1])]
    for d0, d1 in pairs:
        for side, cnt in (("t", "num_node1"), ("s", "num_edge1")):
            if pos:
                x0 = np.asarray(getattr(d0, "pos_" + side), dtype=np.float32).reshape(-1)
            else:
                x0 = np.asarray(getattr(d0, "x_" + side)[:, 0], dtype=np.float32)
            n = x0.size
            n_seg = int(getattr(d1, "x_" + side).shape[0])
            counts = np.asarray(getattr(d0, cnt), dtype=np.int64).reshape(-1)
            ahead = np.zeros(counts.size, dtype=np.float32)
            ahead[1:] = np.cumsum(np.asarray(getattr(d1, cnt), dtype=np.int64).reshape(-1))[:-1]
            per_row = np.zeros(n, dtype=np.float32)
            k = min(int(counts.sum()), n)
            per_row[:k] = np.repeat(ahead, counts)[:k]
            cl = x0 + per_row
            idx = np.where(np.isinf(cl), n_seg, cl).astype(np.int64)
            if idx.size and (idx.min() < 0 or idx.max() > n_seg):
                raise ValueError(f"pool_tables: cluster ids outside [0, {n_seg}] on side {side}")
            order = np.argsort(idx, kind="stable")
            rowptr = np.zeros(n_seg + 2, dtype=np.int32)
            rowptr[1:] = np.cumsum(np.bincount(idx, minlength=n_seg + 1)).astype(np.int32)
            setattr(d0, "pool_rowptr_" + side, torch.from_numpy(rowptr))
            setattr(d0, "pool_rows_" + side, torch.from_numpy(order.astype(np.int32)))


def level_caps(levels: Sequence[Sequence["Batch"]], quantum: int = 512) -> List[Dict[str, int]]:
    out = []
    for lv in zip(*levels):
        cs = [static_caps(b, quantum) for b in lv]
        out.append({k: max(c[k] for c in cs) for k in cs[0]})
    return out


def pad_levels(datas: Sequence["Batch"], caps: Sequence[Dict[str, int]]) -> List["Batch"]:
    if len(datas) != len(caps):
        raise ValueError("pad_levels: one caps dict per level")
    out = [pad_batch(b, c) for b, c in zip(datas, caps)]
    p0, b0 = out[0], datas[0]
    for key in ("x_t", "x_s"):
        x = getattr(p0, key).clone()
        x[getattr(b0, key).size(0):, 0] = float("inf")
        setattr(p0, key, x)
    if getattr(b0, "pool_rowptr_t", None) is not None and p0.x_t.device.type == "cpu":
        pool_tables(out)
    else:
        for k in ("pool_rowptr_t", "pool_rows_t", "pool_rowptr_s", "pool_rows_s"):
            if hasattr(p0, k):
                delattr(p0, k)
    return out


def _h2d(a: np.ndarray, dev: torch.device) -> torch.Tensor:
    t = torch.from_numpy(np.ascontiguousarray(a))
    if torch.device(dev).type != "cuda":
        return t
    return t.pin_memory().to(dev, non_blocking=True)


def pad_batch(b: "Batch", caps: Dict[str, int]) -> "Batch":
    nt, ns = b.x_t.size(0), b.x_s.size(0)
    Rt, Rs = caps["rows_t"], caps["rows_s"]
    dev = b.x_t.device
    if Rt <= nt or Rs <= ns:
        raise ValueError(f"pad_batch: caps ({Rt}, {Rs}) must exceed the rows ({nt}, {ns})")
    out = Batch()
    for k, v in vars(b).items():
        setattr(out, k, v)
    out.l1_factor = getattr(b, "l1_factor", False)
    for k in list(vars(out)):
        if k.startswith(tuple(_HALO_KEYS)) or k.startswith("halo_bounds"):
            delattr(out, k)

    def pad_rows(x, R):
        return torch.cat([x, x.new_zeros((R - x.size(0),) + tuple(x.shape[1:]))], 0)

    def pad_coo(ei, w, n, R, Z):
        extra = Z - ei.size(1)
        if extra < 0:
            raise ValueError(f"pad_batch: {ei.size(1)} Laplacian entries exceed the cap {Z}")
        per_row = _spread(extra, R - n)
        rows = _h2d(np.repeat(np.arange(n, R), per_row).astype(np.int64), ei.device).to(ei.dtype)
        return (torch.cat([ei, torch.stack([rows, rows])], 1),
                torch.cat([w, w.new_zeros(extra)]), per_row)

    out.x_t, out.x_s = pad_rows(b.x_t, Rt), pad_rows(b.x_s, Rs)
    y = getattr(b, "y", None)
    if torch.is_tensor(y) and y.dim() >= 1 and getattr(b, "num_graphs", None) != y.size(0):
        if y.size(0) == ns:
            out.y = pad_rows(y, Rs)
        elif y.size(0) == nt:
            out.y = pad_rows(y, Rt)
    out.edge_index_t, out.edge_weight_t, _ = pad_coo(b.edge_index_t, b.edge_weight_t, nt, Rt,
                                                        caps["nnz_t"])
    out.edge_index_s, out.edge_weight_s, _ = pad_coo(b.edge_index_s, b.edge_weight_s, ns, Rs,
                                                        caps["nnz_s"])
    if getattr(b, "csr_rowptr_t", None) is not None or getattr(b, "csr_rowptr_s", None) is not None:
        _attach_csr(out)
    if getattr(b, "edge_index", None) is not None:
        nodes = _h2d((nt + np.arange(Rs - ns) % (Rt - nt)).astype(np.int64),
                     b.edge_index.device).to(b.edge_index.dtype)
        out.edge_index = torch.cat([b.edge_index, torch.stack([nodes, nodes])], 1)
        if getattr(b, "inc_rowptr", None) is not None:
            out.inc_rowptr, out.inc_eids = incidence_csr(out.edge_index, Rt)
            out.deg_t, out.inv_deg_t = node_degree(out.inc_rowptr, valid=nt)
            if out.l1_factor and getattr(b, "fac_alpha", None) is not None:
                factor_tables(out)
    for side, n, R in (("t", nt, Rt), ("s", ns, Rs)):
        o = getattr(b, "row_order_" + side, None)
        if o is not None:
            setattr(out, "row_order_" + side,
                    torch.cat([o, torch.arange(n, R, dtype=o.dtype, device=o.device)]))
        setattr(out, "n_valid_" + side, torch.full((1,), n, dtype=torch.int32, device=dev))
    out.valid_mask_t = torch.arange(Rt, device=dev) < nt
    out.num_nodes = Rt
    if dev.type == "cuda":
        out._mark()
    return out


ARENA_ALIGN = 256


def arena_alloc(shapes: Dict[str, tuple], pin: bool = False, device=None):
    offs, off = {}, 0
    for k, (shape, dt) in shapes.items():
        nb = int(np.prod(shape)) * torch.empty((), dtype=dt).element_size()
        offs[k] = (off, nb)
        off += (nb + ARENA_ALIGN - 1) // ARENA_ALIGN * ARENA_ALIGN
    arena = torch.empty(max(off, 1), dtype=torch.uint8, pin_memory=pin, device=device)
    views = {k: arena[o:o + nb].view(shapes[k][1]).view(shapes[k][0])
             for k, (o, nb) in offs.items()}
    return arena, views


class PackedGraphs:

    _KEYS = ("x_t", "x_s", "edge_index_t", "edge_weight_t", "edge_index_s", "edge_weight_s",
             "edge_index")

    def __init__(self, graphs: Sequence[PairData], check_hodge: bool = True):
        from . import _lib
        self._lib = _lib
        G = len(graphs)
        if G == 0:
            raise ValueError("PackedGraphs: no graphs")
        for g in graphs:
            for k in self._KEYS:
                if getattr(g, k, None) is None:
                    raise ValueError(f"PackedGraphs: graph without {k}")
        a = lambda v, dt: np.ascontiguousarray(np.asarray(v), dtype=dt)
        self.f_t = int(graphs[0].x_t.shape[1])
        self.f_s = int(graphs[0].x_s.shape[1])
        if any(g.x_t.shape[1] != self.f_t or g.x_s.shape[1] != self.f_s for g in graphs):
            raise ValueError("PackedGraphs: feature widths differ between graphs")
        cnt = lambda f: np.concatenate([[0], np.cumsum([f(g) for g in graphs])]).astype(np.int64)
        self.node_ptr = cnt(lambda g: g.x_t.shape[0])
        self.edge_ptr = cnt(lambda g: g.x_s.shape[0])
        self.lt_ptr = cnt(lambda g: np.asarray(g.edge_index_t).shape[1])
        self.ls_ptr = cnt(lambda g: np.asarray(g.edge_index_s).shape[1])
        for g in graphs:
            if np.asarray(g.edge_index).shape[1] != g.x_s.shape[0]:
                raise ValueError("PackedGraphs: edge_index must have one column per x_s row")
        self.x_t = np.concatenate([a(g.x_t, np.float32) for g in graphs])
        self.x_s = np.concatenate([a(g.x_s, np.float32) for g in graphs])
        cat = lambda k, i, dt: np.concatenate([a(getattr(g, k), np.int64)[i].astype(dt)
                                               for g in graphs])
        self.lt_row, self.lt_col = cat("edge_index_t", 0, np.int32), cat("edge_index_t", 1, np.int32)
        self.ls_row, self.ls_col = cat("edge_index_s", 0, np.int32), cat("edge_index_s", 1, np.int32)
        self.b1_src, self.b1_dst = cat("edge_index", 0, np.int32), cat("edge_index", 1, np.int32)
        self.lt_w = np.concatenate([a(g.edge_weight_t, np.float32).reshape(-1) for g in graphs])
        self.ls_w = np.concatenate([a(g.edge_weight_s, np.float32).reshape(-1) for g in graphs])
        ys = [getattr(g, "y", None) for g in graphs]
        if all(y is not None for y in ys):
            self.y = np.stack([a(y, np.float32).reshape(-1) for y in ys])
            self.y_dim = int(self.y.shape[1])
            self._y_dtype = torch.as_tensor(ys[0]).dtype
        else:
            self.y, self.y_dim, self._y_dtype = np.zeros((G, 0), np.float32), 0, None
        if self._y_dtype is not None and self._y_dtype != torch.float32:
            raise ValueError("PackedGraphs: y must be float32")
        if check_hodge:
            sorted_sym = {k: all(is_sorted_symmetric(np.asarray(getattr(g, k)),
                                                     np.asarray(getattr(g, w)))
                                 for g in graphs)
                          for k, w in (("edge_index_s", "edge_weight_s"),
                                       ("edge_index_t", "edge_weight_t"))}
        else:
            ok = all(getattr(g, "_hodge_sorted", False) for g in graphs)
            sorted_sym = {"edge_index_s": ok, "edge_index_t": ok}
        if not all(sorted_sym.values()):
            raise ValueError("PackedGraphs: every Laplacian COO must be row-sorted and symmetric "
                             "(the Hodge builder's dense_to_sparse output)")
        self.hodge_sorted = sorted_sym
        self.n_graphs = G
        self._desc = _lib.PackedGraphsDesc(
            G, self.node_ptr.ctypes.data, self.edge_ptr.ctypes.data, self.lt_ptr.ctypes.data,
            self.ls_ptr.ctypes.data, self.x_t.ctypes.data, self.f_t, self.x_s.ctypes.data,
            self.f_s, self.lt_row.ctypes.data, self.lt_col.ctypes.data, self.lt_w.ctypes.data,
            self.ls_row.ctypes.data, self.ls_col.ctypes.data, self.ls_w.ctypes.data,
            self.b1_src.ctypes.data, self.b1_dst.ctypes.data, self.y.ctypes.data, self.y_dim)

    def __len__(self) -> int:
        return self.n_graphs

    def graph(self, i: int) -> PairData:
        n0, n1 = self.node_ptr[i], self.node_ptr[i + 1]
        e0, e1 = self.edge_ptr[i], self.edge_ptr[i + 1]
        t0, t1 = self.lt_ptr[i], self.lt_ptr[i + 1]
        s0, s1 = self.ls_ptr[i], self.ls_ptr[i + 1]
        T = lambda v: torch.from_numpy(np.ascontiguousarray(v))
        ei = lambda r, c: T(np.stack([r, c]).astype(np.int64))
        return PairData(edge_index_s=ei(self.ls_row[s0:s1], self.ls_col[s0:s1]),
                        x_s=T(self.x_s[e0:e1]), edge_index_t=ei(self.lt_row[t0:t1],
                                                               self.lt_col[t0:t1]),
                        x_t=T(self.x_t[n0:n1]), edge_weight_s=T(self.ls_w[s0:s1]),
                        edge_weight_t=T(self.lt_w[t0:t1]),
                        edge_index=ei(self.b1_src[e0:e1], self.b1_dst[e0:e1]),
                        y=T(self.y[i]) if self.y_dim else None)

    def _factor_ok(self, i: int) -> bool:
        cache = self.__dict__.setdefault("_fac", {})
        if i not in cache:
            g = self.graph(i)
            cache[i] = hodge_factor_ok(g.edge_index, g.x_t.shape[0], g.edge_index_s,
                                       g.edge_weight_s)
        return cache[i]

    def sizes(self, idx) -> Tuple[int, int, int, int]:
        idx = np.ascontiguousarray(idx, dtype=np.int64)
        out = np.zeros(4, dtype=np.int64)
        self._lib.check(self._lib.LIB.hlhgat_collate_sizes(C_ref(self._desc), idx.ctypes.data,
                                                           idx.size, out.ctypes.data),
                        "collate_sizes")
        return tuple(int(v) for v in out)

    def caps_for(self, idx, quantum: int = 512) -> Dict[str, int]:
        n_t, n_s, z_t, z_s = self.sizes(idx)
        return {"rows_t": _roundup(n_t + PAD_MIN_ROWS, quantum),
                "rows_s": _roundup(n_s + PAD_MIN_ROWS, quantum),
                "nnz_t": _roundup(z_t + 1, 4 * quantum), "nnz_s": _roundup(z_s + 1, 4 * quantum)}

    def collate(self, idx, caps: Optional[Dict[str, int]] = None, pin: bool = False) -> "Batch":
        idx = np.ascontiguousarray(idx, dtype=np.int64)
        B = int(idx.size)
        n_t, n_s, z_t, z_s = self.sizes(idx)
        padded = caps is not None
        Rt, Rs = (caps["rows_t"], caps["rows_s"]) if padded else (n_t, n_s)
        Zt, Zs = (caps["nnz_t"], caps["nnz_s"]) if padded else (z_t, z_s)
        if padded and (Rt <= n_t or Rs <= n_s):
            raise ValueError(f"PackedGraphs.collate: caps ({Rt}, {Rs}) must exceed the rows "
                             f"({n_t}, {n_s})")
        if padded and (Zt < z_t or Zs < z_s):
            raise ValueError(f"PackedGraphs.collate: {z_t} / {z_s} Laplacian entries exceed "
                             f"the caps {Zt} / {Zs}")
        f32, i32, i64 = torch.float32, torch.int32, torch.int64
        shapes = {"x_t": ((Rt, self.f_t), f32), "x_s": ((Rs, self.f_s), f32),
                  "edge_index_t": ((2, Zt), i64), "edge_weight_t": ((Zt,), f32),
                  "edge_index_s": ((2, Zs), i64), "edge_weight_s": ((Zs,), f32),
                  "edge_index": ((2, Rs), i64), "y": ((B * self.y_dim,), f32),
                  "num_node1": ((B,), i64), "num_edge1": ((B,), i64),
                  "csr_rowptr_t": ((Rt + 1,), i32), "csr_col_t": ((Zt,), i32),
                  "csr_rowptr_s": ((Rs + 1,), i32), "csr_col_s": ((Zs,), i32),
                  "inc_rowptr": ((Rt + 1,), i32), "inc_eids": ((2 * Rs,), i32),
                  "deg_t": ((Rt,), f32), "inv_deg_t": ((Rt,), f32),
                  "seg_ptr_t": ((B + 1,), i32), "seg_ptr_s": ((B + 1,), i32),
                  "valid_mask_t": ((Rt,), torch.bool),
                  "n_valid_t": ((1,), i32), "n_valid_s": ((1,), i32)}
        arena, t = arena_alloc(shapes, pin)
        o = self._lib.CollatedDesc(Rt, Rs, Zt, Zs, *[t[k].data_ptr() for k in (
            "x_t", "x_s", "edge_index_t", "edge_weight_t", "edge_index_s", "edge_weight_s",
            "edge_index", "y", "num_node1", "num_edge1", "csr_rowptr_t", "csr_col_t",
            "csr_rowptr_s", "csr_col_s", "inc_rowptr", "inc_eids", "deg_t", "inv_deg_t",
            "seg_ptr_t", "seg_ptr_s", "valid_mask_t")], 0, 0)
        self._lib.check(self._lib.LIB.hlhgat_collate(C_ref(self._desc), idx.ctypes.data, B,
                                                     C_ref(o)), "collate")
        b = Batch()
        b.num_graphs = B
        for k in self._KEYS:
            setattr(b, k, t[k])
        if self.y_dim:
            b.y = t["y"]
        b.num_node1, b.num_edge1 = t["num_node1"], t["num_edge1"]
        b.num_nodes = Rt
        b.hodge_sorted = dict(self.hodge_sorted)
        b.l1_factor = (not padded and z_s >= FACTOR_MIN_ROW * n_s and n_s > 0
                       and all(self._factor_ok(int(i)) for i in idx))
        for k in ("csr_rowptr_t", "csr_col_t", "csr_rowptr_s", "csr_col_s", "inc_rowptr",
                  "inc_eids", "deg_t", "inv_deg_t", "seg_ptr_t", "seg_ptr_s"):
            setattr(b, k, t[k])
        if padded:
            t["n_valid_t"][0] = n_t
            t["n_valid_s"][0] = n_s
            b.n_valid_t = t["n_valid_t"]
            b.n_valid_s = t["n_valid_s"]
            b.valid_mask_t = t["valid_mask_t"]
        b._arena = arena
        return b


def C_ref(struct):
    import ctypes
    return ctypes.byref(struct)


class BoundaryOperator:

    _MM = None

    def __init__(self, edge_index: torch.Tensor, num_node: int, num_edge: int,
                 _transposed: bool = False, _absolute: bool = False, _base=None):
        self.edge_index = edge_index
        self.num_node = int(num_node)
        self.num_edge = int(num_edge)
        if edge_index.size(1) != self.num_edge:
            raise ValueError(f"adj2par1: edge_index has {edge_index.size(1)} edges, "
                             f"num_edge={num_edge}")
        self.transposed = bool(_transposed)
        self.absolute = bool(_absolute)
        self._base = _base
        self._inc = None
        self.valid_t = getattr(edge_index, "_hlhgat_valid_t", None)
        self.valid_s = getattr(edge_index, "_hlhgat_valid_s", None)

    @property
    def shape(self):
        return (torch.Size([self.num_edge, self.num_node]) if self.transposed
                else torch.Size([self.num_node, self.num_edge]))

    def size(self, dim: Optional[int] = None):
        return self.shape if dim is None else self.shape[dim]

    def dim(self) -> int:
        return 2

    is_sparse = True
    layout = torch.sparse_coo
    dtype = torch.float32

    @property
# ... 309 lines not shown
```

hl-hgat_amd/hlhgat/ops.py:

```python
from __future__ import annotations

import contextlib
import ctypes as C
import math
import os
import weakref
from dataclasses import dataclass
from typing import Tuple, List, Optional, Sequence

import torch

from . import _lib
from ._lib import LIB, check

try:
    from . import _hlhgat_ext as _ext
except ImportError as e:
    raise ImportError(f"hlhgat: torch extension _hlhgat_ext missing ({e}); run the build "
                      f"(make -C hl-hgat_amd/csrc)") from e

__all__ = [
    "SparseCSR", "HodgeOperator", "Incidence", "hodge_operator", "incidence",
    "mark_hodge", "set_row_mask", "refresh_row_mask", "simplex_keep",
    "spmm", "poly_basis", "hodge_poly_conv", "linear_blocks", "mlp2", "nei_value",
# ... 152 lines not shown
    def side_context(self):
        return torch.cuda.stream(self.side) if self.on else contextlib.nullcontext()

    def to_main(self, *ts):
        if self.on:
            for t in _tensors(ts):
                t.record_stream(self.main)
        return ts if len(ts) != 1 else ts[0]

    def __exit__(self, *exc):
        global _CHAIN
        if self.on:
            _ext.set_chain(False)
            _CHAIN = None
            self.main.wait_stream(self.side)
        return False


def active_chains(device):
    ch = _CHAIN
    if ch is None or device is None or ch.device != device:
        return None
    return ch


def fork(fn_main, fn_side, side_inputs=(), device=None, slot=0):
    if not _FORK_ENABLED or device is None or device.type != "cuda":
        return fn_main(), fn_side()
    main = torch.cuda.current_stream(device)
    side = side_stream(device, slot)
    side.wait_stream(main)
    with torch.cuda.stream(side):
        for t in _tensors(side_inputs):
            t.record_stream(side)
        out_side = fn_side()
    out_main = fn_main()
    main.wait_stream(side)
    for t in _tensors(out_side):
        t.record_stream(main)
    return out_main, out_side


@dataclass
class SparseCSR:
    rowptr: torch.Tensor
    col: torch.Tensor
    val: Optional[torch.Tensor]
    n_rows: int
    n_cols: int
    nnz: int
    order: Optional[torch.Tensor] = None
    valid: Optional[torch.Tensor] = None
    halo: Optional[tuple] = None


@dataclass
class HodgeOperator:
    fwd: SparseCSR
    bwd: SparseCSR
    factor: Optional[tuple] = None
    factor_nodes: int = 0
    masked_from: Optional[tuple] = None


@dataclass
class Incidence:
    rowptr: torch.Tensor
    edge_ids: torch.Tensor
    edge_index: torch.Tensor
    n_nodes: int
    n_edges: int


class _IdCache:

    def __init__(self):
        self._d = {}

    def get(self, key_tensors: Sequence[torch.Tensor], extra):
        k = (tuple(id(t) for t in key_tensors), extra)
        hit = self._d.get(k)
        if hit is None:
            return None
        versions, value = hit
        if versions != tuple(t._version for t in key_tensors):
            return None
        return value

    def put(self, key_tensors: Sequence[torch.Tensor], extra, value):
        k = (tuple(id(t) for t in key_tensors), extra)
        self._d[k] = (tuple(t._version for t in key_tensors), value)
        for t in key_tensors:
            weakref.finalize(t, self._d.pop, k, None)
        return value

    def clear(self):
        self._d.clear()


_HODGE_CACHE = _IdCache()
_INC_CACHE = _IdCache()
_RCP_CACHE = _IdCache()


def clear_caches() -> None:
    _HODGE_CACHE.clear()
# ... 287 lines not shown
    rowptr = torch.empty(n_rows + 1, dtype=torch.int32, device=dev)
    col32 = torch.empty(max(nnz, 1), dtype=torch.int32, device=dev)[:nnz]
    val = (torch.empty(max(nnz, 1), dtype=torch.float32, device=dev)[:nnz]
           if w is not None else None)
    ws_bytes = int(LIB.hlhgat_csr_workspace_bytes(nnz))
    ws = torch.empty(ws_bytes, dtype=torch.uint8, device=dev)
    check(LIB.hlhgat_csr_from_coo(row.data_ptr() if nnz else None,
                                  col.data_ptr() if nnz else None, _ptr(w), nnz, n_rows,
                                  max(n_cols, 1), rowptr.data_ptr(),
                                  col32.data_ptr() if nnz else None, _ptr(val) if nnz else None,
                                  None, ws.data_ptr(), ws_bytes, _stream(row)),
          "csr_from_coo")
    return SparseCSR(rowptr, col32, val, n_rows, n_cols, nnz)


def hodge_operator(edge_index: torch.Tensor, edge_weight: Optional[torch.Tensor],
                   n: int) -> HodgeOperator:
    bound = getattr(edge_index, "_hlhgat_row_mask", None)
    if bound is not None:
        return _masked_operator(edge_index, edge_weight, n, bound, refresh=False)
    return _hodge_operator(edge_index, edge_weight, n)


def _hodge_operator(edge_index: torch.Tensor, edge_weight: Optional[torch.Tensor],
                    n: int) -> HodgeOperator:
    _req_dev(edge_index, "edge_index", torch.int64)
    if edge_index.dim() != 2 or edge_index.size(0) != 2:
        raise RuntimeError(f"hlhgat: edge_index must be [2, nnz] (got {tuple(edge_index.shape)})")
    if edge_weight is not None:
        _req_dev(edge_weight, "edge_weight")
        if edge_weight.numel() != edge_index.size(1):
            raise RuntimeError("hlhgat: edge_weight must have one entry per edge")
    keys = [edge_index] + ([edge_weight] if edge_weight is not None else [])
    hit = _HODGE_CACHE.get(keys, n)
    if hit is not None:
        return hit
    ei = edge_index.contiguous()
    w = edge_weight.contiguous() if edge_weight is not None else None
    order = getattr(edge_index, "_hlhgat_row_order", None)
    if order is not None and order.numel() != n:
        raise RuntimeError(f"hlhgat: row schedule has {order.numel()} entries, operator {n} rows")
    valid = getattr(edge_index, "_hlhgat_valid", None)
    if getattr(edge_index, "_hlhgat_sorted_symmetric", False):
        pre = getattr(edge_index, "_hlhgat_csr", None)
        if pre is not None and pre[0].numel() == n + 1 and pre[1].numel() == ei.size(1):
            a = SparseCSR(pre[0], pre[1], w, n, n, ei.size(1))
        else:
            a = _csr_sorted(ei[0], ei[1], w, n, n)
        a.order = order
        a.valid = valid
        halo = getattr(edge_index, "_hlhgat_halo", None)
        if halo is not None:
            _attach_halo(a, halo)
        op = HodgeOperator(a, a)
        decl = getattr(edge_index, "_hlhgat_factor", None)
        if decl is not None and FACTOR_ENABLED and w is not None:
            _build_factor(op, ei, w, decl)
    else:
        fwd = _csr_general(ei[1], ei[0], w, n, n)
        bwd = _csr_general(ei[0], ei[1], w, n, n)
        for c in (fwd, bwd):
            c.order = order
            c.valid = valid
        op = HodgeOperator(fwd, bwd)
    return _HODGE_CACHE.put(keys, n, op)


def set_row_mask(edge_index: torch.Tensor, mask: Optional[torch.Tensor]) -> torch.Tensor:
    if mask is None:
        if hasattr(edge_index, "_hlhgat_row_mask"):
            del edge_index._hlhgat_row_mask
        return edge_index
    if not getattr(edge_index, "_hlhgat_sorted_symmetric", False):
        raise RuntimeError("hlhgat: set_row_mask needs a sorted symmetric Laplacian "
                           "(mark_hodge); a general operator cannot take a row mask")
    _req_dev(edge_index, "edge_index", torch.int64)
    _req_dev(mask, "mask")
    if mask.dim() != 1 or not mask.is_contiguous() or mask.device != edge_index.device:
        raise RuntimeError(f"hlhgat: mask must be a contiguous 1-D tensor on {edge_index.device} "
                           f"(got {tuple(mask.shape)} on {mask.device})")
    bound = getattr(edge_index, "_hlhgat_row_mask", None)
    if bound is None or bound[0] is not mask:
        edge_index._hlhgat_row_mask = (mask, {})
    return edge_index


def refresh_row_mask(edge_index: torch.Tensor, edge_weight: torch.Tensor,
                     n: int) -> HodgeOperator:
    bound = getattr(edge_index, "_hlhgat_row_mask", None)
    if bound is None:
        raise RuntimeError("hlhgat: refresh_row_mask: no mask bound (set_row_mask)")
    return _masked_operator(edge_index, edge_weight, n, bound, refresh=True)


def _masked_operator(edge_index, edge_weight, n: int, bound, refresh: bool) -> HodgeOperator:
    mask, bufs = bound
    if edge_weight is None:
        raise RuntimeError("hlhgat: a row-masked operator needs edge weights")
    if mask.numel() != n:
        raise RuntimeError(f"hlhgat: row mask has {mask.numel()} entries, operator {n} rows")
    keys, extra = [edge_index, edge_weight], (n, "row_mask", id(mask))
    op = _HODGE_CACHE.get(keys, extra)
    fresh = op is None
    if fresh:
        base = _hodge_operator(edge_index, edge_weight, n)
        a = base.fwd
# ... 43 lines not shown
def simplex_thresholds(aug_prob: float, p: float, jitter: float) -> Tuple[int, int, int]:
    for name, v in (("aug_prob", aug_prob), ("p", p), ("jitter", jitter)):
        if not 0.0 <= float(v) <= 1.0:
            raise ValueError(f"simplex dropout: {name} has to be between 0 and 1, but got {v}")
    Ta, Tp, Tj = (int(math.floor(float(v) * 16777216.0)) for v in (aug_prob, p, jitter))
    if Tp + Tj > 1 << 24:
        raise ValueError(f"simplex dropout: p + jitter = {p} + {jitter} exceeds 1")
    return Ta, Tp, Tj


def simplex_keep(seg_ptr: torch.Tensor, mask: torch.Tensor, aug_prob: float, p: float,
                 jitter: float, site: int = 0, protect: Optional[torch.Tensor] = None,
                 column: Optional[torch.Tensor] = None) -> torch.Tensor:
    _req_dev(mask, "mask")
    _req_dev(seg_ptr, "seg_ptr", torch.int32)
    if mask.dim() != 1 or not mask.is_contiguous() or seg_ptr.dim() != 1 or seg_ptr.numel() < 1 \
            or not seg_ptr.is_contiguous():
        raise RuntimeError("hlhgat: simplex_keep: mask [n_rows] and seg_ptr [G + 1] must be "
                           "contiguous 1-D tensors")
    n = mask.numel()
    for name, t in (("protect", protect), ("column", column)):
        if t is None:
            continue
        _req_dev(t, name)
        if t.dim() == 2 and t.size(1) == 1:
            t = t[:, 0]
        if t.dim() != 1 or t.numel() != n or (n > 1 and t.stride(0) < 1):
            raise RuntimeError(f"hlhgat: simplex_keep: {name} must be a [n_rows] (strided) view "
                               f"(got {tuple(t.shape)})")
        if name == "protect":
            protect = t
        else:
            column = t
    if not 0 <= int(site) < (1 << 30):
        raise ValueError(f"simplex dropout: site {site} out of range")
    Ta, Tp, Tj = simplex_thresholds(aug_prob, p, jitter)
    st = _dropout_st(mask.device)
    ld = lambda t: max(int(t.stride(0)), 1)
    check(LIB.hlhgat_simplex_keep(
        seg_ptr.data_ptr(), seg_ptr.numel() - 1, n, _ptr(protect),
        ld(protect) if protect is not None else 0, Ta, Tp, Tj, SIMPLEX_SITE + 2 * int(site),
        st.dev.data_ptr(), mask.data_ptr(), _ptr(column), ld(column) if column is not None else 0,
        _stream(mask)), "simplex_keep")
    return mask


def set_csr(edge_index: torch.Tensor, rowptr: torch.Tensor, col: torch.Tensor) -> torch.Tensor:
    edge_index._hlhgat_csr = (
        rowptr.to(device=edge_index.device, dtype=torch.int32).contiguous(),
        col.to(device=edge_index.device, dtype=torch.int32).contiguous())
    return edge_index


def set_incidence(edge_index: torch.Tensor, rowptr: torch.Tensor,
                  edge_ids: torch.Tensor) -> torch.Tensor:
    edge_index._hlhgat_incidence = (
        rowptr.to(device=edge_index.device, dtype=torch.int32).contiguous(),
        edge_ids.to(device=edge_index.device, dtype=torch.int32).contiguous())
    return edge_index


def incidence(edge_index: torch.Tensor, n_nodes: int) -> Incidence:
    _req_dev(edge_index, "edge_index", torch.int64)
    hit = _INC_CACHE.get([edge_index], n_nodes)
    if hit is not None:
        return hit
    ei = edge_index.contiguous()
    E = ei.size(1)
    dev = ei.device
    pre = getattr(edge_index, "_hlhgat_incidence", None)
    if pre is not None:
        rowptr, eids = pre
        if rowptr.numel() != n_nodes + 1 or eids.numel() != 2 * E:
            raise RuntimeError(f"hlhgat: attached incidence CSR has {rowptr.numel() - 1} rows / "
                               f"{eids.numel()} entries, expected {n_nodes} / {2 * E}")
        inc = Incidence(rowptr, eids, ei, n_nodes, E)
        signs = getattr(edge_index, "_hlhgat_inc_signs", None)
        if torch.is_tensor(signs) and signs.numel() == 2 * E and signs.device == dev:
            inc._signs = signs
        return _INC_CACHE.put([edge_index], n_nodes, inc)
    rowptr = torch.empty(n_nodes + 1, dtype=torch.int32, device=dev)
    eids = torch.empty(max(2 * E, 1), dtype=torch.int32, device=dev)[:2 * E]
    ws_bytes = int(LIB.hlhgat_csr_workspace_bytes(2 * E))
    ws = torch.empty(ws_bytes, dtype=torch.uint8, device=dev)
    check(LIB.hlhgat_incidence_csr(ei.data_ptr() if E else None, E, n_nodes,
                                   rowptr.data_ptr(), eids.data_ptr() if E else None,
                                   ws.data_ptr(), ws_bytes, _stream(ei)),
          "incidence_csr")
    return _INC_CACHE.put([edge_index], n_nodes, Incidence(rowptr, eids, ei, n_nodes, E))


def _poly_step(A: SparseCSR, X: torch.Tensor, Y: torch.Tensor, *, rs=None, Z=None, P=None,
               Q=None, alpha=1.0, beta=0.0, gamma=0.0, div=1.0, p=0.0, q=0.0) -> None:
    d = X.size(1)
    check(LIB.hlhgat_poly_step(
        A.rowptr.data_ptr(), A.col.data_ptr() if A.nnz else None, _ptr(A.val) if A.nnz else None,
        _ptr(rs), A.n_rows, A.nnz, _ptr(A.order), _halo_desc(A), X.data_ptr(), _ld(X), d,
        _ptr(Z), _ld(Z) if Z is not None else 0, _ptr(P), _ld(P) if P is not None else 0,
        _ptr(Q), _ld(Q) if Q is not None else 0, alpha, beta, gamma, div, p, q,
        Y.data_ptr(), _ld(Y), _stream(X)), "poly_step")


def spmm(A: SparseCSR, X: torch.Tensor) -> torch.Tensor:
    _req_dev(X, "X")
    X = _rows2d(X, "X")
    Y = torch.empty(A.n_rows, X.size(1), device=X.device, dtype=X.dtype)
# ... 41 lines not shown
                   dAs: List[torch.Tensor], accumulate=False) -> None:
    nb = len(Ws)
    check(LIB.hlhgat_proj_bwd_data(
        nb, G.data_ptr(), _ld(G), _arr(C.c_void_p, [w.data_ptr() for w in Ws]),
        _arr(C.c_int64, [w.stride(0) for w in Ws]), _arr(C.c_int64, kbs), G.size(0), G.size(1),
        _arr(C.c_void_p, [d.data_ptr() for d in dAs]), _arr(C.c_int64, [_ld(d) for d in dAs]),
        int(accumulate), _stream(G)), "proj_bwd_data")


def _proj_bwd_weight(G: torch.Tensor, As: List[torch.Tensor], dWs: List[torch.Tensor],
                     dbias: Optional[torch.Tensor]) -> None:
    nb = len(As)
    kb = _arr(C.c_int64, [a.size(1) for a in As])
    M, N = G.size(0), G.size(1)
    wsf = int(LIB.hlhgat_proj_bwd_weight_workspace_floats(nb, kb, M, N, int(dbias is not None)))
    ws = torch.empty(max(wsf, 1), device=G.device, dtype=torch.float32)
    check(LIB.hlhgat_proj_bwd_weight(
        nb, G.data_ptr(), _ld(G), _arr(C.c_void_p, [a.data_ptr() for a in As]),
        _arr(C.c_int64, [_ld(a) for a in As]), kb, M, N,
        _arr(C.c_void_p, [d.data_ptr() for d in dWs]), _arr(C.c_int64, [d.stride(0) for d in dWs]),
        _ptr(dbias), 0, ws.data_ptr(), wsf, _stream(G)), "proj_bwd_weight")


def _bn_args(bn: Optional[torch.nn.BatchNorm1d]):
    track = bn.training and bn.track_running_stats and bn.running_mean is not None
    if track and bn.momentum is None:
        momentum = 1.0 / float(bn.num_batches_tracked.item() + 1)
    else:
        momentum = float(bn.momentum) if bn.momentum is not None else 0.0
    return (bn.weight, bn.bias, bn.running_mean if track else None,
            bn.running_var if track else None, bn.num_batches_tracked if track else None,
            momentum, float(bn.eps))


def _bn_uses_batch_stats(bn) -> bool:
    return bn.training or not bn.track_running_stats


def hodge_poly_conv(x: torch.Tensor, op: HodgeOperator, weights: Sequence[torch.Tensor],
                    bias: Optional[torch.Tensor], kind: int = POLY_LAGUERRE,
                    bn: Optional[torch.nn.BatchNorm1d] = None, relu: bool = False,
                    out: Optional[torch.Tensor] = None) -> torch.Tensor:
    _req_dev(x, "x")
    if x.size(0) != op.fwd.n_rows:
        raise RuntimeError(f"hlhgat: x has {x.size(0)} rows but the operator has "
                           f"{op.fwd.n_rows}")
    A, At = op.fwd, op.bwd
    ws = list(weights)
    if bn is not None and x.dim() == 2 and _bn_uses_batch_stats(bn) and sync_bn_group(bn) is None:
        if x.size(0) < 2 and bn.training:
            raise ValueError("Expected more than 1 value per channel when training")
        return _ext.conv_bn(x, A.rowptr, A.col, A.val, At.rowptr, At.col, At.val, A.nnz, kind,
                            ws, bias, *_bn_args(bn), 2 if relu else 1, out, A.order, At.order,
                            A.valid, *_halo_args(A), *_factor_args(op))
    sink = out if (bn is None and not relu and x.dim() == 2) else None
    y = _ext.conv_bn(x, A.rowptr, A.col, A.val, At.rowptr, At.col, At.val, A.nnz, kind, ws,
                     bias, None, None, None, None, None, 0.0, 0.0, 0, sink, A.order, At.order,
                     A.valid, *_halo_args(A), *_factor_args(op))
    if bn is not None:
        y = batch_norm_act(y, bn, relu, valid=A.valid)
    elif relu:
        y = torch.relu(y)
    return y


DENSE_SLAB = True
GRAD_SINK = True


class DenseConcat:

    def __init__(self, rows: int, width: int, like: torch.Tensor):
        self.S = torch.empty(rows, width, dtype=torch.float32, device=like.device)
        self.width = width
        self._state = _DenseGrad(self.S)
        self.parts: List[torch.Tensor] = []
        self.cols: List[Tuple[int, int]] = []
        self.owned: List[bool] = []

    @property
    def used(self) -> int:
        return self.cols[-1][1] if self.cols else 0

    def sink(self, w: int) -> torch.Tensor:
        c0 = self.used
        if c0 + w > self.width:
            raise RuntimeError(f"hlhgat: DenseConcat overflow ({c0}+{w} > {self.width})")
        return self.S[:, c0:c0 + w]

    def append(self, y: torch.Tensor) -> None:
        if y.dim() != 2 or y.size(0) != self.S.size(0):
            raise RuntimeError(f"hlhgat: DenseConcat rows {self.S.size(0)}, got {tuple(y.shape)}")
        c0 = self.used
        c1 = c0 + y.size(1)
        if c1 > self.width:
            raise RuntimeError(f"hlhgat: DenseConcat overflow ({c1} > {self.width})")
        if y.data_ptr() != self.S.data_ptr() + 4 * c0 or y.stride(0) != self.S.stride(0):
            self.S.data[:, c0:c1].copy_(y.detach())
        self.parts.append(y)
        self.cols.append((c0, c1))
        self.owned.append(False)

    def grad_sink(self) -> Optional[torch.Tensor]:
        if (not GRAD_SINK or not torch.is_grad_enabled()
                or not any(p.requires_grad for p in self.parts)):
            return None
        if self._state.G is None:
            self._state.G = torch.empty_like(self.S)
            self._state.sink = True
        return self._state.G[:, :self.used], self._state.written

# ... 1624 lines not shown
```

include/hlhgat.h:

```cpp
#ifndef HLHGAT_H_
#define HLHGAT_H_

#include <stddef.h>
#include <stdint.h>

#ifdef __cplusplus
extern "C" {
#endif

#define HLHGAT_OK 0
#define HLHGAT_EINVAL 1
#define HLHGAT_EHIP 2

#define HLHGAT_POLY_LAGUERRE 0
#define HLHGAT_POLY_CHEB 1
#define HLHGAT_POLY_LAGUERRE_DEMO 2

#define HLHGAT_SIGMA_SIGMOID 0
#define HLHGAT_SIGMA_RELU 1

int hlhgat_version(void);
const char* hlhgat_last_error(void);

size_t hlhgat_csr_workspace_bytes(int64_t nnz);
// ... 17 lines not shown
                         int64_t n_nodes, int32_t* rowptr, int32_t* edge_ids,
                         void* workspace, size_t workspace_bytes, void* stream);

typedef struct hlhgat_halo {
  const int32_t* hdr;
  const int32_t* tile_ptr;
  const int32_t* halo_ptr;
  const int32_t* halo;
  const int32_t* srp;
  const uint16_t* lcol;
  const float* sval;
  int64_t n_tiles;
  int32_t max_halo;
  int32_t max_rows;
  int32_t max_nnz;
} hlhgat_halo_t;

int hlhgat_halo_tiles(const int32_t* rowptr, const int32_t* col, int64_t n_rows,
                      int64_t n_cols, const int32_t* order, int32_t max_rows,
                      int32_t max_nnz, int32_t max_halo, int32_t* tile_ptr,
                      int32_t* halo_ptr, int32_t* halo, int32_t* srp, uint16_t* lcol,
                      int32_t* eperm, int32_t* hdr, int64_t* n_tiles, int64_t* n_halo);

int hlhgat_graclus(const int64_t* edge_index, const double* weight, int64_t n_edges,
                   int64_t n_nodes, const int64_t* perm, int64_t* cluster);
int hlhgat_mlgc_map(const int64_t* cluster, int64_t n_nodes, const int64_t* edge_index,
                    int64_t n_edges, int64_t* c_node, float* c_edge, int64_t* coarse_edges,
                    int64_t* n_coarse_nodes, int64_t* n_coarse_edges);
int hlhgat_mlgc_batch(int64_t n_graphs, const int64_t* node_ptr, const int64_t* edge_ptr,
                      const int64_t* edges, const int64_t* perm, int n_threads, int64_t* c_node,
                      float* c_edge, int64_t* coarse_edges, int64_t* coarse_n,
                      int64_t* coarse_e);

typedef struct {
  int64_t n_graphs;
  const int64_t* node_ptr;
  const int64_t* edge_ptr;
  const int64_t* lt_ptr;
  const int64_t* ls_ptr;
  const float* x_t;
  int64_t f_t;
  const float* x_s;
  int64_t f_s;
  const int32_t* lt_row;
  const int32_t* lt_col;
  const float* lt_w;
  const int32_t* ls_row;
  const int32_t* ls_col;
  const float* ls_w;
  const int32_t* b1_src;
  const int32_t* b1_dst;
  const float* y;
  int64_t y_dim;
} hlhgat_packed_graphs_t;
typedef struct {
  int64_t rows_t, rows_s, nnz_t, nnz_s;
  float* x_t;
  float* x_s;
  int64_t* edge_index_t;
  float* edge_weight_t;
  int64_t* edge_index_s;
  float* edge_weight_s;
  int64_t* edge_index;
  float* y;
  int64_t* num_node1;
  int64_t* num_edge1;
  int32_t* csr_rowptr_t;
  int32_t* csr_col_t;
  int32_t* csr_rowptr_s;
  int32_t* csr_col_s;
  int32_t* inc_rowptr;
  int32_t* inc_eids;
  float* deg_t;
  float* inv_deg_t;
  int32_t* seg_ptr_t;
  int32_t* seg_ptr_s;
  uint8_t* valid_mask_t;
  int64_t n_t, n_s;
} hlhgat_collated_t;
int hlhgat_collate_sizes(const hlhgat_packed_graphs_t* d, const int64_t* idx, int64_t n_idx,
                         int64_t* sizes);
int hlhgat_collate(const hlhgat_packed_graphs_t* d, const int64_t* idx, int64_t B,
                   hlhgat_collated_t* out);

int hlhgat_gather_f32(const float* src, const int32_t* idx, int64_t n, float* dst,
                      void* stream);

int hlhgat_spmm(const int32_t* rowptr, const int32_t* col, const float* val,
                int64_t n_rows, int64_t nnz, const int32_t* row_order,
                const hlhgat_halo_t* halo, const float* X, int64_t ldx,
                int64_t d, float* Y, int64_t ldy, void* stream);

int hlhgat_poly_step(const int32_t* rowptr, const int32_t* col,
                     const float* val, const float* rs, int64_t n_rows,
                     int64_t nnz, const int32_t* row_order,
                     const hlhgat_halo_t* halo, const float* X,
                     int64_t ldx, int64_t d,
                     const float* Z, int64_t ldz, const float* P, int64_t ldp,
                     const float* Q, int64_t ldq, float alpha, float beta,
                     float gamma, float div, float p, float q, float* Y,
                     int64_t ldy, void* stream);

int hlhgat_incidence_step(const int32_t* rowptr, const int32_t* col, const float* val,
                          const float* rs, int64_t n_rows, int64_t nnz, int64_t n_src,
                          const float* X, int64_t ldx, int64_t d, const float* Z, int64_t ldz,
                          float alpha, float gamma, float* Y, int64_t ldy, void* stream);

int hlhgat_poly_basis_fwd(int kind, const int32_t* rowptr, const int32_t* col,
                          const float* val, int64_t n, int64_t nnz,
                          const int32_t* row_order, const hlhgat_halo_t* halo,
                          const float* X, int64_t ldx, int64_t F, int K, float* T,
                          void* stream);

int hlhgat_poly_basis_bwd(int kind, const int32_t* rowptr_t,
                          const int32_t* col_t, const float* val_t, int64_t n,
                          int64_t nnz, const int32_t* row_order,
                          const hlhgat_halo_t* halo, int64_t F,
                          int K, float* G, void* stream);

typedef struct hlhgat_hodge_factor {
  const int32_t* node_rowptr;
  const int32_t* node_edge;
  const float* node_sign;
  const int32_t* node_order;
  int64_t n_nodes;
  const int32_t* ends;
  const float* alpha;
  const int32_t* edge_order;
  int64_t n_edges;
} hlhgat_hodge_factor_t;

int64_t hlhgat_hodge_factor_work_floats(int64_t n_nodes, int64_t F);

int hlhgat_hodge_spmm(const hlhgat_hodge_factor_t* f, const float* X, int64_t ldx,
                      int64_t d, float* Y, int64_t ldy, float* work, void* stream);

int hlhgat_hodge_poly_step(const hlhgat_hodge_factor_t* f, const float* X, int64_t ldx,
                           int64_t d, const float* Z, int64_t ldz, const float* P, int64_t ldp,
                           const float* Q, int64_t ldq, float alpha, float beta, float gamma,
                           float div, float p, float q, float* Y, int64_t ldy, float* work,
                           void* stream);

int hlhgat_poly_basis_fwd_factored(int kind, const hlhgat_hodge_factor_t* f,
                                   const float* X, int64_t ldx, int64_t F, int K, float* T,
                                   float* work, void* stream);
int hlhgat_poly_basis_bwd_factored(int kind, const hlhgat_hodge_factor_t* f, int64_t F,
                                   int K, float* G, float* work, void* stream);

int64_t hlhgat_hodge_lmax_workspace_bytes(int64_t n_nodes, int steps);
int hlhgat_hodge_lmax(const int32_t* inc_rowptr, const int32_t* inc_edge,
                      const int64_t* edge_index, int64_t n_edges, int64_t n_nodes,
                      const int64_t* node_ptr, int64_t n_graphs, int steps, double* lmax,
                      void* workspace, int64_t workspace_bytes, void* stream);
int64_t hlhgat_eig_pe_workspace_bytes(int64_t n_graphs, int64_t max_nodes, int k);
int hlhgat_eig_pe(const int32_t* inc_rowptr, const int32_t* inc_edge, const int64_t* edge_index,
                  int64_t n_edges, int64_t n_nodes, const int64_t* node_ptr, int64_t n_graphs,
                  int64_t max_nodes, int k, float* pe, int64_t ldpe, double* lmax,
                  void* workspace, int64_t workspace_bytes, void* stream);
int hlhgat_hodge_row_sizes(const int32_t* inc_rowptr, const int64_t* edge_index,
                           int64_t n_edges, int64_t n_nodes, int32_t* sizes_l0,
                           int32_t* sizes_l1, void* stream);
int hlhgat_hodge_build(const int32_t* inc_rowptr, const int32_t* inc_edge,
                       const int64_t* edge_index, int64_t n_edges, int64_t n_nodes,
                       const float* lam_node, const int32_t* rowptr_l0, int32_t* col_l0,
                       float* val_l0, int64_t cap_l0, const int32_t* rowptr_l1,
                       int32_t* col_l1, float* val_l1, int64_t cap_l1, void* stream);

#define HLHGAT_MAX_BLOCKS 16

int hlhgat_proj_fwd(int nblocks, const float* const* A, const int64_t* lda,
                    const float* const* W, const int64_t* ldw,
// ... 356 lines not shown
```

Baseline: 384,500 graphs/s.

## Fuse K=3 Laguerre basis steps using precomputed squared-operator CSR tables

```diff
diff --git a/hl-hgat_amd/csrc/collate.hip b/hl-hgat_amd/csrc/collate.hip
--- a/hl-hgat_amd/csrc/collate.hip
+++ b/hl-hgat_amd/csrc/collate.hip
@@ -1,3 +1,4 @@
+#include <algorithm>
 #include <cstdint>
 #include <cstring>
 #include <vector>
@@ -47,6 +48,108 @@
   for (int64_t e = 0; e < nnz; ++e) ccol[e] = (int32_t)col[e];
 }
 
+int concat_sq(const hlhgat_packed_graphs_t* d, const int64_t* idx, int64_t B,
+              const int64_t* row_ptr, const int64_t* sq_ptr, const int32_t* sq_col,
+              const float* sq_v1, const float* sq_v2, int64_t R, int64_t Z2, int32_t* rowptr2,
+              int32_t* col2, float* v1, float* v2) {
+  int64_t n = 0, z = 0;
+  rowptr2[0] = 0;
+  for (int64_t b = 0; b < B; ++b) {
+    const int64_t r0 = row_ptr[idx[b]], r1 = row_ptr[idx[b] + 1];
+    const int64_t e0 = sq_ptr[r0], e1 = sq_ptr[r1];
+    HLH_CHECK_ARG(e1 >= e0 && z + (e1 - e0) <= Z2 && n + (r1 - r0) <= R,
+                  "collate: squared-operator table of graph %lld exceeds the capacity %lld",
+                  (long long)idx[b], (long long)Z2);
+    for (int64_t r = r0; r < r1; ++r)
+      rowptr2[n + (r - r0) + 1] = (int32_t)(z + (sq_ptr[r + 1] - e0));
+    for (int64_t e = e0; e < e1; ++e) {
+      HLH_CHECK_ARG(sq_col[e] >= 0 && sq_col[e] < r1 - r0,
+                    "collate: squared-operator column out of range in graph %lld",
+                    (long long)idx[b]);
+      col2[z + (e - e0)] = (int32_t)(n + sq_col[e]);
+    }
+    std::memcpy(v1 + z, sq_v1 + e0, sizeof(float) * (size_t)(e1 - e0));
+    std::memcpy(v2 + z, sq_v2 + e0, sizeof(float) * (size_t)(e1 - e0));
+    n += r1 - r0;
+    z += e1 - e0;
+  }
+  for (int64_t r = n; r < R; ++r) rowptr2[r + 1] = (int32_t)z;
+  std::memset(col2 + z, 0, sizeof(int32_t) * (size_t)(Z2 - z));
+  std::memset(v1 + z, 0, sizeof(float) * (size_t)(Z2 - z));
+  std::memset(v2 + z, 0, sizeof(float) * (size_t)(Z2 - z));
+  return HLHGAT_OK;
+}
+
+}
+
+extern "C" int hlhgat_csr_square(const int32_t* rowptr, const int32_t* col, const float* val,
+                                 int64_t n, int32_t* rowptr2, int32_t* col2, float* v1,
+                                 float* v2, int64_t cap, int64_t* nnz2) {
+  HLH_CHECK_ARG(n >= 0 && n < INT32_MAX && rowptr && rowptr2 && nnz2,
+                "csr_square: bad arguments");
+  HLH_CHECK_ARG(!col2 || (v1 && v2 && cap >= 0), "csr_square: col2 without v1 / v2");
+  const int64_t nnz = rowptr[n];
+  HLH_CHECK_ARG(rowptr[0] == 0 && nnz >= 0 && (nnz == 0 || (col && val)),
+                "csr_square: bad CSR");
+  for (int64_t i = 0; i < n; ++i) {
+    HLH_CHECK_ARG(rowptr[i + 1] >= rowptr[i] && rowptr[i + 1] <= nnz,
+                  "csr_square: row pointers of row %lld out of order", (long long)i);
+    for (int64_t e = rowptr[i]; e < rowptr[i + 1]; ++e)
+      HLH_CHECK_ARG(col[e] >= 0 && col[e] < n && (e == rowptr[i] || col[e] >= col[e - 1]),
+                    "csr_square: row %lld: column out of range or not ascending", (long long)i);
+  }
+  std::vector<int32_t> slot((size_t)n, -1), cols;
+  std::vector<double> acc;
+  std::vector<float> own;
+  std::vector<int32_t> perm;
+  int64_t z = 0;
+  rowptr2[0] = 0;
+  for (int64_t i = 0; i < n; ++i) {
+    cols.clear();
+    acc.clear();
+    own.clear();
+    auto at = [&](int32_t j) -> int32_t {
+      if (slot[j] < 0) {
+        slot[j] = (int32_t)cols.size();
+        cols.push_back(j);
+        acc.push_back(0.0);
+        own.push_back(0.f);
+      }
+      return slot[j];
+    };
+    for (int64_t e = rowptr[i]; e < rowptr[i + 1]; ++e) {
+      const int32_t s = at(col[e]);
+      own[s] = own[s] + val[e];
+    }
+    for (int64_t e = rowptr[i]; e < rowptr[i + 1]; ++e) {
+      const int32_t k = col[e];
+      const double lik = (double)val[e];
+      for (int64_t f = rowptr[k]; f < rowptr[k + 1]; ++f) {
+        const int32_t s = at(col[f]);
+        acc[s] += lik * (double)val[f];
+      }
+    }
+    const int64_t len = (int64_t)cols.size();
+    HLH_CHECK_ARG(z + len < INT32_MAX, "csr_square: table too large for int32 offsets");
+    if (col2) {
+      HLH_CHECK_ARG(z + len <= cap, "csr_square: table exceeds the capacity %lld",
+                    (long long)cap);
+      perm.resize((size_t)len);
+      for (int64_t u = 0; u < len; ++u) perm[u] = (int32_t)u;
+      std::sort(perm.begin(), perm.end(),
+                [&](int32_t a, int32_t b) { return cols[a] < cols[b]; });
+      for (int64_t u = 0; u < len; ++u) {
+        col2[z + u] = cols[perm[u]];
+        v1[z + u] = own[perm[u]];
+        v2[z + u] = (float)acc[perm[u]];
+      }
+    }
+    for (int32_t j : cols) slot[j] = -1;
+    z += len;
+    rowptr2[i + 1] = (int32_t)z;
+  }
+  *nnz2 = z;
+  return HLHGAT_OK;
 }
 
 extern "C" int hlhgat_collate_sizes(const hlhgat_packed_graphs_t* d, const int64_t* idx,
@@ -186,6 +289,22 @@
   }
   if (o->valid_mask_t)
     for (int64_t r = 0; r < Rt; ++r) o->valid_mask_t[r] = r < nt ? 1 : 0;
+  if (o->sq_rowptr_t && o->sq_col_t && o->sq_v1_t && o->sq_v2_t) {
+    HLH_CHECK_ARG(d->sqt_ptr && d->sqt_col && d->sqt_v1 && d->sqt_v2 && o->nnz2_t >= 0 &&
+                      o->nnz2_t < INT32_MAX,
+                  "collate: no packed L0 squared-operator table");
+    rc = concat_sq(d, idx, B, d->node_ptr, d->sqt_ptr, d->sqt_col, d->sqt_v1, d->sqt_v2, Rt,
+                   o->nnz2_t, o->sq_rowptr_t, o->sq_col_t, o->sq_v1_t, o->sq_v2_t);
+    if (rc) return rc;
+  }
+  if (o->sq_rowptr_s && o->sq_col_s && o->sq_v1_s && o->sq_v2_s) {
+    HLH_CHECK_ARG(d->sqs_ptr && d->sqs_col && d->sqs_v1 && d->sqs_v2 && o->nnz2_s >= 0 &&
+                      o->nnz2_s < INT32_MAX,
+                  "collate: no packed L1 squared-operator table");
+    rc = concat_sq(d, idx, B, d->edge_ptr, d->sqs_ptr, d->sqs_col, d->sqs_v1, d->sqs_v2, Rs,
+                   o->nnz2_s, o->sq_rowptr_s, o->sq_col_s, o->sq_v1_s, o->sq_v2_s);
+    if (rc) return rc;
+  }
   o->n_t = nt;
   o->n_s = ns;
   return HLHGAT_OK;
diff --git a/hl-hgat_amd/csrc/poly.hip b/hl-hgat_amd/csrc/poly.hip
--- a/hl-hgat_amd/csrc/poly.hip
+++ b/hl-hgat_amd/csrc/poly.hip
@@ -193,6 +193,126 @@
 template <int V, int LPR>
 __global__ __launch_bounds__(256) void k_poly_step_deep(PolyArgs a) {
   poly_step_body<V, LPR, 8>(a, blk_hw());
+}
+
+struct PairArgs {
+  const int32_t* order;
+  const int32_t* rowptr;
+  const int32_t* col;
+  const float* v1;
+  const float* v2;
+  const float* A;
+  const float* B;
+  const float* C;
+  float* Y0;
+  float* Y1;
+  int64_t lda, ldb, ldc, ldy0, ldy1;
+  int64_t n_rows;
+  int d;
+};
+
+template <bool ADJ>
+struct PairDepth {
+  static constexpr int value = ADJ ? 4 : 8;
+};
+
+template <int V, int LPR, bool ADJ>
+__device__ __forceinline__ void poly_pair_body(const PairArgs& a, Blk blk) {
+  using vt = typename VecT<V>::type;
+  constexpr int NB = PairDepth<ADJ>::value;
+  const int64_t slot = ((int64_t)xcd_slot(blk.x, blk.gx) * 256 + threadIdx.x) / LPR;
+  const int sub = threadIdx.x % LPR;
+  const bool live = slot < a.n_rows;
+  const int64_t row = live ? (a.order ? (int64_t)a.order[slot] : slot) : 0;
+  const int e0 = live ? a.rowptr[row] : 0;
+  const int e1 = live ? a.rowptr[row + 1] : 0;
+  const float* __restrict__ A = a.A;
+  const float* __restrict__ B = a.B;
+  for (int f0 = 0; f0 < a.d; f0 += LPR * V) {
+    const int f = f0 + sub * V;
+    const bool fok = live && f < a.d;
+    vt s1, s2, s3;
+#pragma unroll
+    for (int i = 0; i < V; ++i) vget(s1, i) = vget(s2, i) = vget(s3, i) = 0.f;
+    for (int eb = e0; eb < e1; eb += LPR) {
+      const int me = eb + sub;
+      const int cm = me < e1 ? a.col[me] : 0;
+      const float w1m = me < e1 ? a.v1[me] : 0.f;
+      const float w2m = me < e1 ? a.v2[me] : 0.f;
+      const int cnt = e1 - eb < LPR ? e1 - eb : LPR;
+      for (int j = 0; j < cnt; j += NB) {
+        const int rem = cnt - j;
+        int c[NB];
+        bool in1[NB];
+#pragma unroll
+        for (int u = 0; u < NB; ++u) {
+          c[u] = __shfl(cm, j + u, LPR);
+          in1[u] = !ADJ || __shfl(w1m, j + u, LPR) != 0.f;
+        }
+        vt xa[NB], xb[NB];
+#pragma unroll
+        for (int u = 0; u < NB; ++u) {
+#pragma unroll
+          for (int i = 0; i < V; ++i) vget(xa[u], i) = vget(xb[u], i) = 0.f;
+          if (fok && u < rem) {
+            if (in1[u]) xa[u] = vload<V>(A + (int64_t)c[u] * a.lda + f);
+            if (ADJ) xb[u] = vload<V>(B + (int64_t)c[u] * a.ldb + f);
+          }
+        }
+#pragma unroll
+        for (int u = 0; u < NB; ++u) {
+          const float w1 = __shfl(w1m, j + u, LPR);
+          const float w2 = __shfl(w2m, j + u, LPR);
+          if (fok && u < rem) {
+#pragma unroll
+            for (int i = 0; i < V; ++i) {
+              vget(s1, i) = vget(s1, i) + w1 * vget(xa[u], i);
+              if (ADJ) {
+                vget(s2, i) = vget(s2, i) + w1 * vget(xb[u], i);
+                vget(s3, i) = vget(s3, i) + w2 * vget(xb[u], i);
+              } else {
+                vget(s2, i) = vget(s2, i) + w2 * vget(xa[u], i);
+              }
+            }
+          }
+        }
+      }
+    }
+    if (!fok) continue;
+    if (ADJ) {
+      vt g0 = vload<V>(a.C + row * a.ldc + f);
+      vt g1 = vload<V>(A + row * a.lda + f);
+      vt g2 = vload<V>(B + row * a.ldb + f);
+      vt dx;
+#pragma unroll
+      for (int i = 0; i < V; ++i) {
+        const float g1p = vget(g1, i) + (3.f * vget(g2, i) - vget(s2, i)) / 2.f;
+        const float lg = vget(s1, i) + (3.f * vget(s2, i) - vget(s3, i)) / 2.f;
+        vget(dx, i) = ((vget(g0, i) + g1p) - lg) - vget(g2, i) / 2.f;
+      }
+      vstore<V>(a.Y0 + row * a.ldy0 + f, dx);
+    } else {
+      vt x = vload<V>(A + row * a.lda + f);
+      vt t1, t2;
+#pragma unroll
+      for (int i = 0; i < V; ++i) {
+        vget(t1, i) = vget(x, i) - vget(s1, i);
+        vget(t2, i) = ((3.f * vget(t1, i) - vget(x, i)) - (vget(s1, i) - vget(s2, i))) / 2.f;
+      }
+      vstore<V>(a.Y0 + row * a.ldy0 + f, t1);
+      vstore<V>(a.Y1 + row * a.ldy1 + f, t2);
+    }
+  }
+}
+
+template <int V, int LPR>
+__global__ __launch_bounds__(256) void k_poly_pair(PairArgs a) {
+  poly_pair_body<V, LPR, false>(a, blk_hw());
+}
+
+template <int V, int LPR>
+__global__ __launch_bounds__(256) void k_poly_pair_adj(PairArgs a) {
+  poly_pair_body<V, LPR, true>(a, blk_hw());
 }
 
 template <int V, int LPR>
@@ -753,9 +873,65 @@
   }
 };
 
+bool& poly_pair_flag() {
+  static bool on = true;
+  return on;
+}
+
+bool pair_usable(const hlhgat_sq_t* sq, int kind, const hlhgat_halo_t* halo,
+                 const hlhgat_hodge_factor_t* fac) {
+  return sq && sq->rowptr && sq->v1 && sq->v2 && (sq->nnz2 == 0 || sq->col) &&
+         poly_pair_flag() && kind == HLHGAT_POLY_LAGUERRE && !fac &&
+         !(halo && halo->lcol && halo->n_tiles > 0);
+}
+
+int launch_pair(PairArgs& a, const hlhgat_sq_t& sq, bool adj, hipStream_t s) {
+  HLH_CHECK_ARG(a.n_rows >= 0 && a.n_rows < (int64_t)INT32_MAX && sq.nnz2 >= 0 &&
+                    sq.nnz2 < (int64_t)INT32_MAX,
+                "poly_pair: sizes out of range");
+  HLH_CHECK_ARG(a.d > 0 && a.A && a.Y0 && (adj ? (a.B && a.C) : a.Y1 != nullptr),
+                "poly_pair: NULL pointer or d <= 0");
+  HLH_CHECK_ARG(a.lda >= a.d && a.ldy0 >= a.d && (adj ? (a.ldb >= a.d && a.ldc >= a.d)
+                                                      : a.ldy1 >= a.d),
+                "poly_pair: ld < d");
+  if (a.n_rows == 0) return HLHGAT_OK;
+  const int v = pick_vec(a.d, {a.lda, a.ldy0, adj ? a.ldb : a.ldy1, adj ? a.ldc : 4},
+                         {a.A, a.Y0, adj ? (const void*)a.B : (const void*)a.Y1, a.C});
+  const int l = pick_lpr(a.d, v);
+  const double bytes = 12.0 * (double)sq.nnz2 + 4.0 * (double)(a.n_rows + 1) +
+                       (adj ? 4.0 : 3.0) * 4.0 * (double)a.n_rows * a.d;
+  ProfScope prof(adj ? HLHGAT_PROF_POLY_ADJ : HLHGAT_PROF_POLY, s, bytes,
+                 (adj ? 6.0 : 4.0) * (double)sq.nnz2 * a.d);
+  if (adj)
+    HLH_DISPATCH_VL(v, l, k_poly_pair_adj, a.n_rows, s, a, &prof);
+  else
+    HLH_DISPATCH_VL(v, l, k_poly_pair, a.n_rows, s, a, &prof);
+  HLH_CHECK_LAUNCH();
+  return HLHGAT_OK;
+}
+
+PairArgs pair_args(const hlhgat_sq_t& sq, const int32_t* order, int64_t n, int64_t d) {
+  PairArgs a{};
+  a.order = order;
+  a.rowptr = sq.rowptr;
+  a.col = sq.col;
+  a.v1 = sq.v1;
+  a.v2 = sq.v2;
+  a.n_rows = n;
+  a.d = (int)d;
+  return a;
+}
+
 }
 
 using namespace hlhgat;
+
+extern "C" int hlhgat_set_poly_pair(int on) {
+  poly_pair_flag() = on != 0;
+  return HLHGAT_OK;
+}
+
+extern "C" int hlhgat_get_poly_pair(void) { return poly_pair_flag() ? 1 : 0; }
 
 extern "C" int hlhgat_spmm(const int32_t* rowptr, const int32_t* col,
                            const float* val, int64_t n_rows, int64_t nnz,
@@ -816,7 +992,8 @@
 int basis_fwd_core(int kind, const int32_t* rowptr, const int32_t* col, const float* val,
                    int64_t n, int64_t nnz, const int32_t* row_order, const hlhgat_halo_t* halo,
                    const float* X, int64_t ldx, int64_t F, int K, float* T,
-                   const hlhgat_hodge_factor_t* fac, float* work, void* stream) {
+                   const hlhgat_hodge_factor_t* fac, float* work, void* stream,
+                   const hlhgat_sq_t* sq = nullptr) {
   HLH_CHECK_ARG(kind == HLHGAT_POLY_LAGUERRE || kind == HLHGAT_POLY_CHEB ||
                     kind == HLHGAT_POLY_LAGUERRE_DEMO,
                 "poly_basis_fwd: bad kind %d", kind);
@@ -827,7 +1004,17 @@
   const StepRunner run{nnz, fac, work, s};
   const int64_t blk = n * F;
   auto Tk = [&](int k) -> float* { return T + (int64_t)(k - 1) * blk; };
-  {
+  const bool pair = K >= 3 && pair_usable(sq, kind, halo, fac);
+  if (pair) {
+    PairArgs a = pair_args(*sq, row_order, n, F);
+    a.A = X;
+    a.lda = ldx;
+    a.Y0 = Tk(1);
+    a.Y1 = Tk(2);
+    a.ldy0 = a.ldy1 = F;
+    int rc = launch_pair(a, *sq, false, s);
+    if (rc) return rc;
+  } else {
     PolyArgs a = make_args(rowptr, col, val, n, X, ldx, F, Tk(1), F, row_order, halo);
     if (kind != HLHGAT_POLY_CHEB) {
       a.alpha = -1.f;
@@ -836,7 +1023,7 @@
     int rc = run(a);
     if (rc) return rc;
   }
-  for (int k = 1; k + 1 < K; ++k) {
+  for (int k = pair ? 2 : 1; k + 1 < K; ++k) {
     const float* prev = (k == 1) ? X : Tk(k - 1);
     const int64_t ldprev = (k == 1) ? ldx : F;
     PolyArgs a = make_args(rowptr, col, val, n, Tk(k), F, F, Tk(k + 1), F, row_order, halo);
@@ -869,7 +1056,8 @@
 int basis_bwd_core(int kind, const int32_t* rowptr_t, const int32_t* col_t,
                    const float* val_t, int64_t n, int64_t nnz, const int32_t* row_order,
                    const hlhgat_halo_t* halo, int64_t F, int K, float* G,
-                   const hlhgat_hodge_factor_t* fac, float* work, void* stream) {
+                   const hlhgat_hodge_factor_t* fac, float* work, void* stream,
+                   const hlhgat_sq_t* sq = nullptr) {
   HLH_CHECK_ARG(kind == HLHGAT_POLY_LAGUERRE || kind == HLHGAT_POLY_CHEB ||
                     kind == HLHGAT_POLY_LAGUERRE_DEMO,
                 "poly_basis_bwd: bad kind %d", kind);
@@ -892,6 +1080,15 @@
     a.p = 1.f;
     return run(a);
   }
+  if (K == 3 && pair_usable(sq, kind, halo, fac)) {
+    PairArgs a = pair_args(*sq, row_order, n, F);
+    a.A = Gk(1);
+    a.B = Gk(2);
+    a.C = Gk(0);
+    a.Y0 = Gk(0);
+    a.lda = a.ldb = a.ldc = a.ldy0 = F;
+    return launch_pair(a, *sq, true, s);
+  }
   for (int k = K - 1; k >= 1; --k) {
     PolyArgs a = make_args(rowptr_t, col_t, val_t, n, Gk(k), F, F, Gk(k - 1), F, row_order, halo);
     a.P = Gk(k - 1);
@@ -933,6 +1130,24 @@
                                      int64_t F, int K, float* G, void* stream) {
   return basis_bwd_core(kind, rowptr_t, col_t, val_t, n, nnz, row_order, halo, F, K, G,
                         nullptr, nullptr, stream);
+}
+
+extern "C" int hlhgat_poly_basis_fwd_sq(int kind, const int32_t* rowptr, const int32_t* col,
+                                        const float* val, int64_t n, int64_t nnz,
+                                        const int32_t* row_order, const hlhgat_halo_t* halo,
+                                        const hlhgat_sq_t* sq, const float* X, int64_t ldx,
+                                        int64_t F, int K, float* T, void* stream) {
+  return basis_fwd_core(kind, rowptr, col, val, n, nnz, row_order, halo, X, ldx, F, K, T,
+                        nullptr, nullptr, stream, sq);
+}
+
+extern "C" int hlhgat_poly_basis_bwd_sq(int kind, const int32_t* rowptr_t, const int32_t* col_t,
+                                        const float* val_t, int64_t n, int64_t nnz,
+                                        const int32_t* row_order, const hlhgat_halo_t* halo,
+                                        const hlhgat_sq_t* sq, int64_t F, int K, float* G,
+                                        void* stream) {
+  return basis_bwd_core(kind, rowptr_t, col_t, val_t, n, nnz, row_order, halo, F, K, G,
+                        nullptr, nullptr, stream, sq);
 }
 
 extern "C" int64_t hlhgat_hodge_factor_work_floats(int64_t n_nodes, int64_t F) {
diff --git a/hl-hgat_amd/csrc/runtime.hip b/hl-hgat_amd/csrc/runtime.hip
--- a/hl-hgat_amd/csrc/runtime.hip
+++ b/hl-hgat_amd/csrc/runtime.hip
@@ -73,7 +73,7 @@
 
 using namespace hlhgat;
 
-extern "C" int hlhgat_version(void) { return 107; }
+extern "C" int hlhgat_version(void) { return 108; }
 
 extern "C" int hlhgat_device_errors(unsigned* out) {
   HLH_CHECK_ARG(out, "device_errors: NULL pointer");
diff --git a/hl-hgat_amd/csrc/torch_ext.cpp b/hl-hgat_amd/csrc/torch_ext.cpp
--- a/hl-hgat_amd/csrc/torch_ext.cpp
+++ b/hl-hgat_amd/csrc/torch_ext.cpp
@@ -609,6 +609,7 @@
   OptT h_hdr;
   std::vector<Tensor> fac;
   int64_t fac_nodes = 0;
+  OptT sq_rowptr, sq_col, sq_v1, sq_v2;
 };
 
 struct ConvDims {
@@ -616,13 +617,14 @@
 };
 struct ConvSaved {
   Tensor x2, T, t_order, valid, t_rowptr, t_col, t_val, pre, yout, mean, invstd, bn_w, bias,
-      bn_b, h_tile, h_ptr, h_cols, h_srp, h_lcol, h_sval, h_hdr;
+      bn_b, h_tile, h_ptr, h_cols, h_srp, h_lcol, h_sval, h_hdr, sq_rowptr, sq_col, sq_v1, sq_v2;
   std::vector<Tensor> W, fac;
   ConvDims d{};
   std::vector<int64_t> xshape, h_bounds;
   std::vector<Tensor*> slots() {
     return {&x2, &T, &t_order, &valid, &t_rowptr, &t_col, &t_val, &pre, &yout, &mean, &invstd,
-            &bn_w, &bias, &bn_b, &h_tile, &h_ptr, &h_cols, &h_srp, &h_lcol, &h_sval, &h_hdr};
+            &bn_w, &bias, &bn_b, &h_tile, &h_ptr, &h_cols, &h_srp, &h_lcol, &h_sval, &h_hdr,
+            &sq_rowptr, &sq_col, &sq_v1, &sq_v2};
   }
   void save(AutogradContext* ctx) {
     ctx->saved_data["dims"] = pod_ints(d);
@@ -677,7 +679,31 @@
   em.opt(c.h_hdr);
   em.list(c.fac);
   em.other();
+  em.opt(c.sq_rowptr);
+  em.opt(c.sq_col);
+  em.opt(c.sq_v1);
+  em.opt(c.sq_v2);
   return p;
+}
+
+hlhgat_sq_t make_sq(const Tensor& rowptr, const Tensor& col, const Tensor& v1, const Tensor& v2,
+                    int64_t n) {
+  for (const Tensor* t : {&rowptr, &col, &v1, &v2})
+    TORCH_CHECK(t->is_cuda() && t->is_contiguous() && t->device() == rowptr.device(),
+                "hlhgat: squared-operator table must be contiguous device tensors");
+  TORCH_CHECK(rowptr.scalar_type() == at::kInt && col.scalar_type() == at::kInt &&
+                  v1.scalar_type() == at::kFloat && v2.scalar_type() == at::kFloat &&
+                  rowptr.numel() == n + 1 && col.numel() == v1.numel() &&
+                  col.numel() == v2.numel(),
+              "hlhgat: squared-operator table must be int32 rowptr [n+1] / col and fp32 v1 / v2 "
+              "of one length");
+  hlhgat_sq_t q{};
+  q.rowptr = rowptr.data_ptr<int>();
+  q.nnz2 = col.numel();
+  q.col = q.nnz2 ? col.data_ptr<int>() : nullptr;
+  q.v1 = v1.data_ptr<float>();
+  q.v2 = v2.data_ptr<float>();
+  return q;
 }
 
 Tensor conv_forward(const ConvArgs& c, ConvSaved& sv) {
@@ -699,6 +725,10 @@
                            has(c.h_sval) ? *c.h_sval : Tensor(), c.h_bounds, *c.h_hdr)
                : hlhgat_halo_t{};
   const bool factored = !c.fac.empty();
+  const bool use_sq = has(c.sq_rowptr) && has(c.sq_col) && has(c.sq_v1) && has(c.sq_v2) &&
+                      !factored && !use_halo && c.nnz > 0 && has(c.a_val);
+  const hlhgat_sq_t sq =
+      use_sq ? make_sq(*c.sq_rowptr, *c.sq_col, *c.sq_v1, *c.sq_v2, N) : hlhgat_sq_t{};
   if (factored && K > 1 && N > 0) {
     const hlhgat_hodge_factor_t hf = make_factor(c.fac, c.fac_nodes, N);
     Tensor work = at::empty({hlhgat_hodge_factor_work_floats(c.fac_nodes, F)}, x.options());
@@ -706,10 +736,12 @@
                                        (int)K, T.data_ptr<float>(), work.data_ptr<float>(), s),
         "poly_basis_fwd_factored");
   } else if (K > 1 && N > 0) {
-    chk(hlhgat_poly_basis_fwd((int)c.kind, c.a_rowptr.data_ptr<int>(),
-                              c.nnz ? c.a_col.data_ptr<int>() : nullptr,
-                              c.nnz ? fptr(c.a_val) : nullptr, N, c.nnz, iptr(c.a_order),
-                              use_halo ? &halo : nullptr, x2.data_ptr<float>(), ld_of(x2), F, (int)K, T.data_ptr<float>(), s),
+    chk(hlhgat_poly_basis_fwd_sq((int)c.kind, c.a_rowptr.data_ptr<int>(),
+                                 c.nnz ? c.a_col.data_ptr<int>() : nullptr,
+                                 c.nnz ? fptr(c.a_val) : nullptr, N, c.nnz, iptr(c.a_order),
+                                 use_halo ? &halo : nullptr, use_sq ? &sq : nullptr,
+                                 x2.data_ptr<float>(), ld_of(x2), F, (int)K, T.data_ptr<float>(),
+                                 s),
         "poly_basis_fwd");
   }
   std::vector<const float*> Ap(K), Wp(K);
@@ -771,6 +803,13 @@
     sv.h_sval = opt_or_undef(c.h_sval);
     sv.h_hdr = *c.h_hdr;
   }
+  if (use_sq && c.t_rowptr.data_ptr() == c.a_rowptr.data_ptr() &&
+      c.t_col.data_ptr() == c.a_col.data_ptr() && fptr(c.t_val) == fptr(c.a_val)) {
+    sv.sq_rowptr = *c.sq_rowptr;
+    sv.sq_col = *c.sq_col;
+    sv.sq_v1 = *c.sq_v1;
+    sv.sq_v2 = *c.sq_v2;
+  }
   sv.W = c.W;
   sv.fac = c.fac;
   std::vector<int64_t> oshape = x.sizes().vec();
@@ -841,11 +880,15 @@
           "poly_basis_bwd_factored");
     } else if (M > 0 && K > 1) {
       const Tensor &tv = sv.t_val, &to = sv.t_order;
-      chk(hlhgat_poly_basis_bwd((int)d.kind, sv.t_rowptr.data_ptr<int>(),
-                                d.nnz ? sv.t_col.data_ptr<int>() : nullptr,
-                                (d.nnz && tv.defined()) ? tv.data_ptr<float>() : nullptr, N, d.nnz,
-                                to.defined() ? to.data_ptr<int>() : nullptr,
-                                use_halo ? &halo : nullptr, F, (int)K, Gs.data_ptr<float>(), s),
+      const bool use_sq = sv.sq_rowptr.defined();
+      const hlhgat_sq_t sq =
+          use_sq ? make_sq(sv.sq_rowptr, sv.sq_col, sv.sq_v1, sv.sq_v2, N) : hlhgat_sq_t{};
+      chk(hlhgat_poly_basis_bwd_sq((int)d.kind, sv.t_rowptr.data_ptr<int>(),
+                                   d.nnz ? sv.t_col.data_ptr<int>() : nullptr,
+                                   (d.nnz && tv.defined()) ? tv.data_ptr<float>() : nullptr, N,
+                                   d.nnz, to.defined() ? to.data_ptr<int>() : nullptr,
+                                   use_halo ? &halo : nullptr, use_sq ? &sq : nullptr, F, (int)K,
+                                   Gs.data_ptr<float>(), s),
           "poly_basis_bwd");
     } else if (M == 0) {
       Gs.zero_();
@@ -864,11 +907,12 @@
                         int64_t bn_mode, OptT out_buf, OptT a_order, OptT t_order, OptT valid,
                         OptT h_tile, OptT h_ptr, OptT h_cols, OptT h_srp, OptT h_lcol,
                         OptT h_sval, std::vector<int64_t> h_bounds, OptT h_hdr,
-                        at::TensorList fac, int64_t fac_nodes) {
+                        at::TensorList fac, int64_t fac_nodes, OptT sq_rowptr, OptT sq_col,
+                        OptT sq_v1, OptT sq_v2) {
     ConvArgs c{x, a_rowptr, a_col, a_val, t_rowptr, t_col, t_val, nnz, kind, W.vec(), bias,
                bn_w, bn_b, bn_rm, bn_rv, bn_nbt, momentum, eps, bn_mode, out_buf, a_order,
                t_order, valid, h_tile, h_ptr, h_cols, h_srp, h_lcol, h_sval, h_bounds, h_hdr,
-               fac.vec(), fac_nodes};
+               fac.vec(), fac_nodes, sq_rowptr, sq_col, sq_v1, sq_v2};
     ConvSaved sv;
     Tensor y = conv_forward(c, sv);
     EdgeMap em;
@@ -1714,11 +1758,11 @@
                int64_t bn_mode, OptT out_buf, OptT a_order, OptT t_order, OptT valid,
                OptT h_tile, OptT h_ptr, OptT h_cols, OptT h_srp, OptT h_lcol, OptT h_sval,
                std::vector<int64_t> h_bounds, OptT h_hdr, std::vector<Tensor> fac,
-               int64_t fac_nodes) {
+               int64_t fac_nodes, OptT sq_rowptr, OptT sq_col, OptT sq_v1, OptT sq_v2) {
   return ConvBNFn::apply(x, a_rowptr, a_col, a_val, t_rowptr, t_col, t_val, nnz, kind,
                          at::TensorList(W), bias, bn_w, bn_b, bn_rm, bn_rv, bn_nbt, momentum, eps,
                          bn_mode, out_buf, a_order, t_order, valid, h_tile, h_ptr, h_cols, h_srp, h_lcol, h_sval, h_bounds,
-                         h_hdr, at::TensorList(fac), fac_nodes);
+                         h_hdr, at::TensorList(fac), fac_nodes, sq_rowptr, sq_col, sq_v1, sq_v2);
 }
 
 Tensor bn_act(Tensor x, OptT w, OptT b, OptT rm, OptT rv, OptT nbt, double momentum, double eps,
diff --git a/hl-hgat_amd/hlhgat/_lib.py b/hl-hgat_amd/hlhgat/_lib.py
--- a/hl-hgat_amd/hlhgat/_lib.py
+++ b/hl-hgat_amd/hlhgat/_lib.py
@@ -47,6 +47,13 @@
                                       c_vp, c_i64, c_i64, c_i32, c_vp, c_vp]),
     "hlhgat_poly_basis_bwd": (c_i32, [c_i32, c_vp, c_vp, c_vp, c_i64, c_i64, c_vp, c_vp,
                                       c_i64, c_i32, c_vp, c_vp]),
+    "hlhgat_poly_basis_fwd_sq": (c_i32, [c_i32, c_vp, c_vp, c_vp, c_i64, c_i64, c_vp, c_vp, c_vp,
+                                         c_vp, c_i64, c_i64, c_i32, c_vp, c_vp]),
+    "hlhgat_poly_basis_bwd_sq": (c_i32, [c_i32, c_vp, c_vp, c_vp, c_i64, c_i64, c_vp, c_vp, c_vp,
+                                         c_i64, c_i32, c_vp, c_vp]),
+    "hlhgat_set_poly_pair": (c_i32, [c_i32]),
+    "hlhgat_get_poly_pair": (c_i32, []),
+    "hlhgat_csr_square": (c_i32, [c_vp, c_vp, c_vp, c_i64, c_vp, c_vp, c_vp, c_vp, c_i64, c_vp]),
     "hlhgat_hodge_factor_work_floats": (c_i64, [c_i64, c_i64]),
     "hlhgat_hodge_spmm": (c_i32, [c_vp, c_vp, c_i64, c_i64, c_vp, c_i64, c_vp, c_vp]),
     "hlhgat_hodge_poly_step": (c_i32, [c_vp, c_vp, c_i64, c_i64, c_vp, c_i64, c_vp, c_i64, c_vp,
@@ -255,7 +262,13 @@
                 ("ls_ptr", c_vp), ("x_t", c_vp), ("f_t", c_i64), ("x_s", c_vp), ("f_s", c_i64),
                 ("lt_row", c_vp), ("lt_col", c_vp), ("lt_w", c_vp), ("ls_row", c_vp),
                 ("ls_col", c_vp), ("ls_w", c_vp), ("b1_src", c_vp), ("b1_dst", c_vp),
-                ("y", c_vp), ("y_dim", c_i64)]
+                ("y", c_vp), ("y_dim", c_i64),
+                ("sqt_ptr", c_vp), ("sqt_col", c_vp), ("sqt_v1", c_vp), ("sqt_v2", c_vp),
+                ("sqs_ptr", c_vp), ("sqs_col", c_vp), ("sqs_v1", c_vp), ("sqs_v2", c_vp)]
+
+
+class SqDesc(C.Structure):
+    _fields_ = [("rowptr", c_vp), ("col", c_vp), ("v1", c_vp), ("v2", c_vp), ("nnz2", c_i64)]
 
 
 class CollatedDesc(C.Structure):
@@ -266,7 +279,9 @@
                 ("csr_col_t", c_vp), ("csr_rowptr_s", c_vp), ("csr_col_s", c_vp),
                 ("inc_rowptr", c_vp), ("inc_eids", c_vp), ("deg_t", c_vp), ("inv_deg_t", c_vp),
                 ("seg_ptr_t", c_vp), ("seg_ptr_s", c_vp), ("valid_mask_t", c_vp),
-                ("n_t", c_i64), ("n_s", c_i64)]
+                ("n_t", c_i64), ("n_s", c_i64), ("nnz2_t", c_i64), ("nnz2_s", c_i64),
+                ("sq_rowptr_t", c_vp), ("sq_col_t", c_vp), ("sq_v1_t", c_vp), ("sq_v2_t", c_vp),
+                ("sq_rowptr_s", c_vp), ("sq_col_s", c_vp), ("sq_v1_s", c_vp), ("sq_v2_s", c_vp)]
 
 
 class HlhgatError(RuntimeError):
diff --git a/hl-hgat_amd/hlhgat/hodge_dataset.py b/hl-hgat_amd/hlhgat/hodge_dataset.py
--- a/hl-hgat_amd/hlhgat/hodge_dataset.py
+++ b/hl-hgat_amd/hlhgat/hodge_dataset.py
@@ -116,6 +116,9 @@
             if (torch.is_tensor(t) and t.is_cuda and torch.is_tensor(rp) and torch.is_tensor(col)
                     and self.hodge_sorted.get(k, False)):
                 ops.set_csr(t, rp, col)
+                sq = tuple(getattr(self, f + "_" + side, None) for f in _SQ_FIELDS)
+                if all(torch.is_tensor(v) and v.is_cuda for v in sq):
+                    ops.set_sq(t, *sq)
         ip, ie = getattr(self, "inc_rowptr", None), getattr(self, "inc_eids", None)
         if torch.is_tensor(ei) and ei.is_cuda and torch.is_tensor(ip) and torch.is_tensor(ie):
             ops.set_incidence(ei, ip, ie)
@@ -264,6 +267,54 @@
             rp, col = laplacian_csr(ei, x.size(0))
             setattr(b, "csr_rowptr_" + side, rp)
             setattr(b, "csr_col_" + side, col)
+
+
+SQ_TABLES = os.environ.get("HLHGAT_SQ_TABLES", "0") == "1"
+SQ_MAX_ROW = 8.0
+_SQ_FIELDS = ("sq_rowptr", "sq_col", "sq_v1", "sq_v2")
+
+
+def sq_wanted(nnz: int, n: int) -> bool:
+    return nnz <= SQ_MAX_ROW * n
+
+
+def laplacian_square(rowptr, col, val, n: int):
+    from . import _lib
+    rp = np.ascontiguousarray(np.asarray(rowptr), dtype=np.int32)
+    c = np.ascontiguousarray(np.asarray(col), dtype=np.int32)
+    v = np.ascontiguousarray(np.asarray(val), dtype=np.float32).reshape(-1)
+    n = int(n)
+    if rp.size != n + 1 or c.size != v.size or (n and int(rp[-1]) != c.size):
+        raise ValueError("laplacian_square: rowptr / col / val sizes do not match")
+    rp2 = np.zeros(n + 1, dtype=np.int32)
+    z = np.zeros(1, dtype=np.int64)
+    p = lambda a: a.ctypes.data if a.size else None
+    _lib.check(_lib.LIB.hlhgat_csr_square(rp.ctypes.data, p(c), p(v), n, rp2.ctypes.data, None,
+                                          None, None, 0, z.ctypes.data), "csr_square")
+    Z = int(z[0])
+    col2 = np.zeros(max(Z, 1), dtype=np.int32)
+    v1, v2 = np.zeros(max(Z, 1), dtype=np.float32), np.zeros(max(Z, 1), dtype=np.float32)
+    _lib.check(_lib.LIB.hlhgat_csr_square(rp.ctypes.data, p(c), p(v), n, rp2.ctypes.data,
+                                          col2.ctypes.data, v1.ctypes.data, v2.ctypes.data, Z,
+                                          z.ctypes.data), "csr_square")
+    return rp2, col2[:Z], v1[:Z], v2[:Z]
+
+
+def _attach_sq(b, graphs) -> None:
+    if not SQ_TABLES:
+        return
+    for side in ("t", "s"):
+        k = "edge_index_" + side
+        rp, col = getattr(b, "csr_rowptr_" + side, None), getattr(b, "csr_col_" + side, None)
+        w = getattr(b, "edge_weight_" + side, None)
+        if rp is None or col is None or w is None or (side == "s" and getattr(b, "l1_factor", False)):
+            continue
+        if not all(sq_wanted(int(np.asarray(getattr(g, k)).shape[1]),
+                             int(getattr(g, "x_" + side).shape[0])) for g in graphs):
+            continue
+        tabs = laplacian_square(rp, col, w, rp.numel() - 1)
+        for f, a in zip(_SQ_FIELDS, tabs):
+            setattr(b, f + "_" + side, torch.from_numpy(np.ascontiguousarray(a)))
 
 
 FACTOR_TABLES = os.environ.get("HLHGAT_FACTOR_TABLES", "1") != "0"
@@ -340,6 +391,7 @@
     for side in ("s", "t"):
         _collate_halo(b, graphs, side)
     _attach_csr(b)
+    _attach_sq(b, graphs)
     ei = getattr(b, "edge_index", None)
     if torch.is_tensor(ei) and torch.is_tensor(getattr(b, "x_t", None)):
         b.inc_rowptr, b.inc_eids = incidence_csr(ei, b.x_t.size(0))
@@ -421,6 +473,9 @@
     caps = {"rows_t": rows_t, "rows_s": rows_s,
             "nnz_t": _roundup(b.edge_index_t.size(1) + 1, 4 * quantum),
             "nnz_s": _roundup(b.edge_index_s.size(1) + 1, 4 * quantum)}
+    for side in ("t", "s"):
+        c = getattr(b, "sq_col_" + side, None)
+        caps["nnz2_" + side] = _roundup(c.numel() + 1, 4 * quantum) if torch.is_tensor(c) else 0
     return caps
 
 
@@ -523,6 +578,20 @@
                                                         caps["nnz_s"])
     if getattr(b, "csr_rowptr_t", None) is not None or getattr(b, "csr_rowptr_s", None) is not None:
         _attach_csr(out)
+    for side, n, R in (("t", nt, Rt), ("s", ns, Rs)):
+        rp, Z2 = getattr(b, "sq_rowptr_" + side, None), int(caps.get("nnz2_" + side, 0) or 0)
+        if rp is None or Z2 <= 0:
+            for f in _SQ_FIELDS:
+                if hasattr(out, f + "_" + side):
+                    delattr(out, f + "_" + side)
+            continue
+        z2 = getattr(b, "sq_col_" + side).numel()
+        if z2 > Z2:
+            raise ValueError(f"pad_batch: {z2} squared-operator entries exceed the cap {Z2}")
+        setattr(out, "sq_rowptr_" + side, torch.cat([rp, rp[-1:].expand(R - n)]))
+        for f in _SQ_FIELDS[1:]:
+            v = getattr(b, f + "_" + side)
+            setattr(out, f + "_" + side, torch.cat([v, v.new_zeros(Z2 - z2)]))
     if getattr(b, "edge_index", None) is not None:
         nodes = _h2d((nt + np.arange(Rs - ns) % (Rt - nt)).astype(np.int64),
                      b.edge_index.device).to(b.edge_index.dtype)
@@ -565,8 +634,10 @@
     _KEYS = ("x_t", "x_s", "edge_index_t", "edge_weight_t", "edge_index_s", "edge_weight_s",
              "edge_index")
 
-    def __init__(self, graphs: Sequence[PairData], check_hodge: bool = True):
+    def __init__(self, graphs: Sequence[PairData], check_hodge: bool = True,
+                 sq_tables: Optional[bool] = None):
         from . import _lib
+        self.sq_tables = SQ_TABLES if sq_tables is None else bool(sq_tables)
         self._lib = _lib
         G = len(graphs)
         if G == 0:
@@ -620,12 +691,53 @@
                              "(the Hodge builder's dense_to_sparse output)")
         self.hodge_sorted = sorted_sym
         self.n_graphs = G
-        self._desc = _lib.PackedGraphsDesc(
-            G, self.node_ptr.ctypes.data, self.edge_ptr.ctypes.data, self.lt_ptr.ctypes.data,
+        self.sqt_ok, self.sqt_ptr, self.sqt_col, self.sqt_v1, self.sqt_v2 = self._pack_sq(
+            self.lt_row, self.lt_col, self.lt_w, self.node_ptr, self.lt_ptr)
+        self.sqs_ok, self.sqs_ptr, self.sqs_col, self.sqs_v1, self.sqs_v2 = self._pack_sq(
+            self.ls_row, self.ls_col, self.ls_w, self.edge_ptr, self.ls_ptr)
+        self._desc = self._make_desc()
+
+    def _pack_sq(self, row, col, w, row_ptr, ent_ptr, chunk: int = 1 << 24):
+        G = self.n_graphs
+        n_g, z_g = np.diff(row_ptr), np.diff(ent_ptr)
+        ok = (z_g <= SQ_MAX_ROW * n_g) & self.sq_tables
+        ptr = np.zeros(int(row_ptr[-1]) + 1, dtype=np.int64)
+        cols, v1s, v2s = [], [], []
+        g0 = 0 if self.sq_tables else G
+        while g0 < G:
+            g1 = max(g0 + 1, int(np.searchsorted(ent_ptr, ent_ptr[g0] + chunk, "right")) - 1)
+            g1 = min(g1, G)
+            r0, r1, e0, e1 = row_ptr[g0], row_ptr[g1], ent_ptr[g0], ent_ptr[g1]
+            gid = np.repeat(np.arange(g0, g1), z_g[g0:g1])
+            keep = ok[gid]
+            off = (row_ptr[gid] - r0)[keep]
+            grow, gcol = row[e0:e1][keep] + off, col[e0:e1][keep] + off
+            rp = np.zeros(int(r1 - r0) + 1, dtype=np.int32)
+            if grow.size:
+                np.cumsum(np.bincount(grow, minlength=int(r1 - r0)), out=rp[1:])
+            rp2, c2, v1, v2 = laplacian_square(rp, gcol, w[e0:e1][keep], int(r1 - r0))
+            row_graph = np.repeat(np.arange(g0, g1), n_g[g0:g1])
+            ent_row = np.repeat(np.arange(int(r1 - r0)), np.diff(rp2))
+            cols.append((c2 - (row_ptr[row_graph] - r0)[ent_row]).astype(np.int32))
+            v1s.append(v1)
+            v2s.append(v2)
+            ptr[r0 + 1:r1 + 1] = ptr[r0] + rp2[1:].astype(np.int64)
+            g0 = g1
+        cat = lambda xs, dt: np.ascontiguousarray(
+            np.concatenate(xs + [np.zeros(1, dt)]), dtype=dt)
+        return ok, ptr, cat(cols, np.int32), cat(v1s, np.float32), cat(v2s, np.float32)
+
+    def _make_desc(self):
+        _lib = self._lib
+        sq = [a.ctypes.data for a in (self.sqt_ptr, self.sqt_col, self.sqt_v1, self.sqt_v2,
+                                      self.sqs_ptr, self.sqs_col, self.sqs_v1, self.sqs_v2)]
+        return _lib.PackedGraphsDesc(
+            self.n_graphs, self.node_ptr.ctypes.data, self.edge_ptr.ctypes.data, self.lt_ptr.ctypes.data,
             self.ls_ptr.ctypes.data, self.x_t.ctypes.data, self.f_t, self.x_s.ctypes.data,
             self.f_s, self.lt_row.ctypes.data, self.lt_col.ctypes.data, self.lt_w.ctypes.data,
             self.ls_row.ctypes.data, self.ls_col.ctypes.data, self.ls_w.ctypes.data,
-            self.b1_src.ctypes.data, self.b1_dst.ctypes.data, self.y.ctypes.data, self.y_dim)
+            self.b1_src.ctypes.data, self.b1_dst.ctypes.data, self.y.ctypes.data, self.y_dim,
+            *sq)
 
     def __len__(self) -> int:
         return self.n_graphs
@@ -663,9 +775,27 @@
 
     def caps_for(self, idx, quantum: int = 512) -> Dict[str, int]:
         n_t, n_s, z_t, z_s = self.sizes(idx)
+        z2_t, z2_s = self.sq_sizes(idx, self._l1_factor(idx, n_s, z_s, False))
         return {"rows_t": _roundup(n_t + PAD_MIN_ROWS, quantum),
                 "rows_s": _roundup(n_s + PAD_MIN_ROWS, quantum),
-                "nnz_t": _roundup(z_t + 1, 4 * quantum), "nnz_s": _roundup(z_s + 1, 4 * quantum)}
+                "nnz_t": _roundup(z_t + 1, 4 * quantum), "nnz_s": _roundup(z_s + 1, 4 * quantum),
+                "nnz2_t": 0 if z2_t is None else _roundup(z2_t + 1, 4 * quantum),
+                "nnz2_s": 0 if z2_s is None else _roundup(z2_s + 1, 4 * quantum)}
+
+    def _l1_factor(self, idx, n_s: int, z_s: int, padded: bool) -> bool:
+        return (not padded and z_s >= FACTOR_MIN_ROW * n_s and n_s > 0
+                and all(self._factor_ok(int(i)) for i in idx))
+
+    def sq_sizes(self, idx, l1_factor: bool = False):
+        idx = np.ascontiguousarray(idx, dtype=np.int64)
+        out = []
+        for ok, ptr, rows, fac in ((self.sqt_ok, self.sqt_ptr, self.node_ptr, False),
+                                   (self.sqs_ok, self.sqs_ptr, self.edge_ptr, l1_factor)):
+            if fac or not bool(ok[idx].all()):
+                out.append(None)
+            else:
+                out.append(int((ptr[rows[idx + 1]] - ptr[rows[idx]]).sum()))
+        return tuple(out)
 
     def collate(self, idx, caps: Optional[Dict[str, int]] = None, pin: bool = False) -> "Batch":
         idx = np.ascontiguousarray(idx, dtype=np.int64)
@@ -681,6 +811,15 @@
             raise ValueError(f"PackedGraphs.collate: {z_t} / {z_s} Laplacian entries exceed "
                              f"the caps {Zt} / {Zs}")
         f32, i32, i64 = torch.float32, torch.int32, torch.int64
+        l1_factor = self._l1_factor(idx, n_s, z_s, padded)
+        z2 = dict(zip("ts", self.sq_sizes(idx, l1_factor)))
+        Z2 = {sd: (int(caps.get("nnz2_" + sd, 0) or 0) if padded else z)
+              for sd, z in z2.items() if z is not None}
+        Z2 = {sd: Z for sd, Z in Z2.items() if not padded or Z > 0}
+        for sd, Z in Z2.items():
+            if Z < z2[sd]:
+                raise ValueError(f"PackedGraphs.collate: {z2[sd]} squared-operator entries "
+                                 f"exceed the cap {Z}")
         shapes = {"x_t": ((Rt, self.f_t), f32), "x_s": ((Rs, self.f_s), f32),
                   "edge_index_t": ((2, Zt), i64), "edge_weight_t": ((Zt,), f32),
                   "edge_index_s": ((2, Zs), i64), "edge_weight_s": ((Zs,), f32),
@@ -693,12 +832,19 @@
                   "seg_ptr_t": ((B + 1,), i32), "seg_ptr_s": ((B + 1,), i32),
                   "valid_mask_t": ((Rt,), torch.bool),
                   "n_valid_t": ((1,), i32), "n_valid_s": ((1,), i32)}
+        for sd, Z in Z2.items():
+            R = Rt if sd == "t" else Rs
+            shapes.update({"sq_rowptr_" + sd: ((R + 1,), i32), "sq_col_" + sd: ((Z,), i32),
+                           "sq_v1_" + sd: ((Z,), f32), "sq_v2_" + sd: ((Z,), f32)})
         arena, t = arena_alloc(shapes, pin)
+        sq_ptrs = [t[f + "_" + sd].data_ptr() if sd in Z2 else None
+                   for sd in "ts" for f in _SQ_FIELDS]
         o = self._lib.CollatedDesc(Rt, Rs, Zt, Zs, *[t[k].data_ptr() for k in (
             "x_t", "x_s", "edge_index_t", "edge_weight_t", "edge_index_s", "edge_weight_s",
             "edge_index", "y", "num_node1", "num_edge1", "csr_rowptr_t", "csr_col_t",
             "csr_rowptr_s", "csr_col_s", "inc_rowptr", "inc_eids", "deg_t", "inv_deg_t",
-            "seg_ptr_t", "seg_ptr_s", "valid_mask_t")], 0, 0)
+            "seg_ptr_t", "seg_ptr_s", "valid_mask_t")], 0, 0, Z2.get("t", 0), Z2.get("s", 0),
+            *sq_ptrs)
         self._lib.check(self._lib.LIB.hlhgat_collate(C_ref(self._desc), idx.ctypes.data, B,
                                                      C_ref(o)), "collate")
         b = Batch()
@@ -710,8 +856,10 @@
         b.num_node1, b.num_edge1 = t["num_node1"], t["num_edge1"]
         b.num_nodes = Rt
         b.hodge_sorted = dict(self.hodge_sorted)
-        b.l1_factor = (not padded and z_s >= FACTOR_MIN_ROW * n_s and n_s > 0
-                       and all(self._factor_ok(int(i)) for i in idx))
+        b.l1_factor = l1_factor
+        for sd in Z2:
+            for f in _SQ_FIELDS:
+                setattr(b, f + "_" + sd, t[f + "_" + sd])
         for k in ("csr_rowptr_t", "csr_col_t", "csr_rowptr_s", "csr_col_s", "inc_rowptr",
                   "inc_eids", "deg_t", "inv_deg_t", "seg_ptr_t", "seg_ptr_s"):
             setattr(b, k, t[k])
diff --git a/hl-hgat_amd/hlhgat/ops.py b/hl-hgat_amd/hlhgat/ops.py
--- a/hl-hgat_amd/hlhgat/ops.py
+++ b/hl-hgat_amd/hlhgat/ops.py
@@ -228,6 +228,7 @@
     order: Optional[torch.Tensor] = None
     valid: Optional[torch.Tensor] = None
     halo: Optional[tuple] = None
+    sq: Optional[tuple] = None
 
 
 @dataclass
@@ -621,6 +622,12 @@
         halo = getattr(edge_index, "_hlhgat_halo", None)
         if halo is not None:
             _attach_halo(a, halo)
+        sq = getattr(edge_index, "_hlhgat_sq", None)
+        if sq is not None and pre is not None and a.rowptr is pre[0] and w is not None:
+            if sq[0].numel() != n + 1 or sq[0].device != ei.device:
+                raise RuntimeError(f"hlhgat: attached squared-operator table has "
+                                   f"{sq[0].numel() - 1} rows, operator {n}")
+            a.sq = sq
         op = HodgeOperator(a, a)
         decl = getattr(edge_index, "_hlhgat_factor", None)
         if decl is not None and FACTOR_ENABLED and w is not None:
@@ -770,6 +777,21 @@
     return edge_index
 
 
+def set_sq(edge_index: torch.Tensor, rowptr2: torch.Tensor, col2: torch.Tensor,
+           v1: torch.Tensor, v2: torch.Tensor) -> torch.Tensor:
+    dev = edge_index.device
+    i32 = lambda t: t.to(device=dev, dtype=torch.int32).contiguous()
+    f32 = lambda t: t.to(device=dev, dtype=torch.float32).contiguous()
+    if not (col2.numel() == v1.numel() == v2.numel()):
+        raise RuntimeError("hlhgat: set_sq: col2, v1 and v2 must have one entry each")
+    edge_index._hlhgat_sq = (i32(rowptr2), i32(col2), f32(v1), f32(v2))
+    return edge_index
+
+
+def _sq_args(A: "SparseCSR"):
+    return A.sq if A.sq is not None else (None, None, None, None)
+
+
 def set_incidence(edge_index: torch.Tensor, rowptr: torch.Tensor,
                   edge_ids: torch.Tensor) -> torch.Tensor:
     edge_index._hlhgat_incidence = (
@@ -917,11 +939,11 @@
             raise ValueError("Expected more than 1 value per channel when training")
         return _ext.conv_bn(x, A.rowptr, A.col, A.val, At.rowptr, At.col, At.val, A.nnz, kind,
                             ws, bias, *_bn_args(bn), 2 if relu else 1, out, A.order, At.order,
-                            A.valid, *_halo_args(A), *_factor_args(op))
+                            A.valid, *_halo_args(A), *_factor_args(op), *_sq_args(A))
     sink = out if (bn is None and not relu and x.dim() == 2) else None
     y = _ext.conv_bn(x, A.rowptr, A.col, A.val, At.rowptr, At.col, At.val, A.nnz, kind, ws,
                      bias, None, None, None, None, None, 0.0, 0.0, 0, sink, A.order, At.order,
-                     A.valid, *_halo_args(A), *_factor_args(op))
+                     A.valid, *_halo_args(A), *_factor_args(op), *_sq_args(A))
     if bn is not None:
         y = batch_norm_act(y, bn, relu, valid=A.valid)
     elif relu:
diff --git a/include/hlhgat.h b/include/hlhgat.h
--- a/include/hlhgat.h
+++ b/include/hlhgat.h
@@ -93,6 +93,14 @@
   const int32_t* b1_dst;
   const float* y;
   int64_t y_dim;
+  const int64_t* sqt_ptr;
+  const int32_t* sqt_col;
+  const float* sqt_v1;
+  const float* sqt_v2;
+  const int64_t* sqs_ptr;
+  const int32_t* sqs_col;
+  const float* sqs_v1;
+  const float* sqs_v2;
 } hlhgat_packed_graphs_t;
 typedef struct {
   int64_t rows_t, rows_s, nnz_t, nnz_s;
@@ -118,7 +126,19 @@
   int32_t* seg_ptr_s;
   uint8_t* valid_mask_t;
   int64_t n_t, n_s;
+  int64_t nnz2_t, nnz2_s;
+  int32_t* sq_rowptr_t;
+  int32_t* sq_col_t;
+  float* sq_v1_t;
+  float* sq_v2_t;
+  int32_t* sq_rowptr_s;
+  int32_t* sq_col_s;
+  float* sq_v1_s;
+  float* sq_v2_s;
 } hlhgat_collated_t;
+int hlhgat_csr_square(const int32_t* rowptr, const int32_t* col, const float* val, int64_t n,
+                      int32_t* rowptr2, int32_t* col2, float* v1, float* v2, int64_t cap,
+                      int64_t* nnz2);
 int hlhgat_collate_sizes(const hlhgat_packed_graphs_t* d, const int64_t* idx, int64_t n_idx,
                          int64_t* sizes);
 int hlhgat_collate(const hlhgat_packed_graphs_t* d, const int64_t* idx, int64_t B,
@@ -158,6 +178,25 @@
                           int64_t nnz, const int32_t* row_order,
                           const hlhgat_halo_t* halo, int64_t F,
                           int K, float* G, void* stream);
+
+typedef struct hlhgat_sq {
+  const int32_t* rowptr;
+  const int32_t* col;
+  const float* v1;
+  const float* v2;
+  int64_t nnz2;
+} hlhgat_sq_t;
+int hlhgat_poly_basis_fwd_sq(int kind, const int32_t* rowptr, const int32_t* col,
+                             const float* val, int64_t n, int64_t nnz,
+                             const int32_t* row_order, const hlhgat_halo_t* halo,
+                             const hlhgat_sq_t* sq, const float* X, int64_t ldx, int64_t F,
+                             int K, float* T, void* stream);
+int hlhgat_poly_basis_bwd_sq(int kind, const int32_t* rowptr_t, const int32_t* col_t,
+                             const float* val_t, int64_t n, int64_t nnz,
+                             const int32_t* row_order, const hlhgat_halo_t* halo,
+                             const hlhgat_sq_t* sq, int64_t F, int K, float* G, void* stream);
+int hlhgat_set_poly_pair(int on);
+int hlhgat_get_poly_pair(void);
 
 typedef struct hlhgat_hodge_factor {
   const int32_t* node_rowptr;
```

Result: no change. 381,700 graphs/s (-0.7%).
